# HUBioDataLab/DrugGEN

Hardware: AMD Instinct MI355X
Metric: molecules/sec GAN step (G+D fwd+bwd), N=45 graphs (higher is better)
Workload: dtype f32

## Files before the change

druggen_amd/_lib.py:

```python
from __future__ import annotations

import contextlib
import ctypes
import os
import threading
from ctypes import c_char_p, c_double, c_float, c_int, c_int64, c_size_t, c_void_p

import torch

_PKG = os.path.dirname(os.path.abspath(__file__))
LIB_PATH = os.environ.get("DG_LIB") or os.path.join(_PKG, "lib", "libdruggen_hip.so")

_P = c_void_p


class FFNFwdArgs(ctypes.Structure):
    _fields_ = [(n, _P) for n in ("x", "w1_packed", "b1", "w2_packed", "b2", "gamma", "beta", "y", "h", "relu_bits", "pre_ln",
                                  "mean", "rstd")] + [("R", c_int64), ("eps", c_float)]


class FFNBwdArgs(ctypes.Structure):
    _fields_ = [(n, _P) for n in ("x", "h", "relu_bits", "pre_ln", "mean", "rstd", "gamma", "w1_dgrad_packed", "w2_dgrad_packed",
                                  "dy", "dz_add", "dz", "dh", "dx", "dgamma", "dbeta", "dw1", "db1", "dw2", "db2", "workspace")] + [
        ("workspace_bytes", c_size_t), ("R", c_int64)]


SIGNATURES = {
    "dg_version": (c_int, []),
    "dg_last_error_string": (c_char_p, []),
    "dg_hidden_bytes": (c_size_t, [c_int64, c_int, c_int]),
    "dg_hidden_scale_offset": (c_size_t, [c_int64, c_int]),
    "dg_attn_core_fwd": (c_int, [_P] * 6 + [c_int, c_int, c_int, c_float, c_int, _P]),
    "dg_attn_core_bwd": (c_int, [_P] * 10 + [c_int, c_int, c_int, c_float, c_int, _P]),
    "dg_attn_core_bwd_add": (c_int, [_P] * 11 + [c_int, c_int, c_int, c_float, c_int, _P]),
    "dg_attn_core_bwd2": (c_int, [_P] * 16 + [c_int, c_int, c_int, c_float, c_int, _P]),
    "dg_attn_core_long_workspace_bytes": (c_size_t, [c_int, c_int, c_int]),
    "dg_attn_core_long_fwd": (c_int, [_P] * 6 + [c_int, c_int, c_int, c_float, c_int, _P]),
    "dg_attn_core_long_bwd": (c_int, [_P] * 12 + [c_size_t, c_int, c_int, c_int, c_float, c_int, _P]),
    "dg_attn_core_long_bwd2": (c_int, [_P] * 17 + [c_size_t, c_int, c_int, c_int, c_float, c_int, _P]),
    "dg_attn_half_packed_bytes": (c_size_t, [c_int]),
    "dg_attn_half_pack": (c_int, [_P, _P, _P, c_int, _P]),
    "dg_attn_half_fwd": (c_int, [_P] * 14 + [c_int, c_int, c_int, c_float, c_float, c_int, _P]),
    "dg_attn_half_f32_fwd": (c_int, [_P] * 17 + [c_int, c_int, c_int, c_float, c_float, _P]),
    "dg_attn_half_f32_bwd1_workspace_bytes": (c_size_t, [c_int]),
    "dg_attn_half_f32_bwd1": (c_int, [_P] * 19 + [_P, c_size_t, c_int, c_int, c_int, c_float, _P]),
    "dg_attn_half_bwd_workspace_bytes": (c_size_t, [c_int, c_int]),
    "dg_attn_half_bwd": (c_int, [_P] * 16 + [_P, c_size_t, c_int, c_int, c_int, c_float, c_int, _P]),
    "dg_ln_residual_fwd": (c_int, [_P] * 7 + [c_int64, c_int, c_float, c_int, _P]),
    "dg_ln_workspace_bytes": (c_size_t, [c_int64, c_int]),
    "dg_ln_residual_bwd": (c_int, [_P] * 9 + [_P, c_size_t, c_int64, c_int, c_int, _P]),
    "dg_ln_residual_bwd_add": (c_int, [_P] * 10 + [_P, c_size_t, c_int64, c_int, c_int, _P]),
    "dg_ln_residual_bwd2": (c_int, [_P] * 10 + [_P, c_size_t, c_int64, c_int, c_int, _P]),
    "dg_linear_wgrad_workspace_bytes": (c_size_t, [c_int64, c_int, c_int]),
    "dg_linear_wgrad": (c_int, [_P] * 5 + [_P, c_size_t, c_int64, c_int, c_int, c_int, _P]),
    "dg_row_gemm_packed_bytes": (c_size_t, [c_int, c_int, c_int]),
    "dg_row_gemm_pack": (c_int, [_P, _P, c_int, c_int, c_int, c_int, _P]),
    "dg_row_gemm_mask_words": (c_size_t, [c_int64, c_int, c_int, c_int]),
    "dg_row_gemm": (c_int, [_P] * 3 + [c_int64, c_int, c_int, _P, c_int, _P, _P, _P, _P, _P, _P, _P, _P, c_float, c_int, _P]),
    "dg_linear_wgrad3": (c_int, [_P] * 6 + [_P, c_size_t, c_int64, c_int, _P]),
    "dg_row_gemm_pack3": (c_int, [_P, _P, _P, _P, c_int, c_int, c_int, _P]),
    "dg_row_gemm_lin3": (c_int, [_P] * 5 + [c_int64, _P, _P, _P, c_int, _P]),
    "dg_row_gemm_sum3": (c_int, [_P] * 5 + [c_int64, _P, c_int, _P]),
    "dg_linear_wgrad_batch_begin": (c_int, []),
    "dg_linear_wgrad_batch_end": (c_int, [_P]),
    "dg_launch_pair_begin": (c_int, []),
    "dg_launch_pair_end": (c_int, [_P]),
    "dg_skinny_linear_fwd": (c_int, [_P] * 4 + [c_int64, c_int, c_int, c_int, _P]),
    "dg_skinny_linear_dgrad": (c_int, [_P] * 3 + [c_int64, c_int, c_int, c_int, _P]),
    "dg_skinny_linear_wgrad": (c_int, [_P] * 5 + [c_size_t, c_int64, c_int, c_int, c_int, _P]),
    "dg_embed_node_chain": (c_int, [_P] * 9 + [c_int64, c_int, c_int, _P]),
    "dg_embed_node_bwd": (c_int, [_P] * 8 + [c_int64, c_int, c_int, _P]),
    "dg_head_chain": (c_int, [_P] * 14 + [c_int64, c_int, _P]),
    "dg_head_bwd": (c_int, [_P] * 10 + [c_int64, c_int, _P]),
    "dg_head_wgrad": (c_int, [_P] * 12 + [c_int64, _P]),
    "dg_row_gemm_pack_batch": (c_int, [_P, c_int, c_int, c_int, _P]),
    "dg_row_gemm_ln_bwd_workspace_bytes": (c_size_t, [c_int]),
    "dg_row_gemm_ln_bwd": (c_int, [_P] * 3 + [c_int64, c_int] + [_P] * 7 + [_P, c_size_t, c_int, _P]),
    "dg_row_gemm_ln_bwd_in": (c_int, [_P] * 10 + [_P, c_size_t, c_int64, c_int, c_int, c_int, _P]),
    "dg_edge_ffn_ln_workspace_bytes": (c_size_t, [c_int64, c_int, c_int]),
    "dg_edge_ffn_ln_fwd": (c_int, [_P] * 13 + [c_int64, c_int, c_int, c_float, c_int, _P]),
    "dg_edge_ffn_ln_bwd": (c_int, [_P] * 20 + [_P, c_size_t, c_int64, c_int, c_int, c_int, _P]),
    "dg_edge_ffn_ln_fwd_pair": (c_int, [ctypes.POINTER(FFNFwdArgs), ctypes.POINTER(FFNFwdArgs), c_int, c_int, c_int, _P]),
    "dg_edge_ffn_ln_bwd_pair": (c_int, [ctypes.POINTER(FFNBwdArgs), ctypes.POINTER(FFNBwdArgs), c_int, c_int, c_int, _P]),
    "dg_ffn_f32_packed_bytes": (c_size_t, []),
    "dg_ffn_f32_pack": (c_int, [_P, _P, _P, _P]),
    "dg_ffn_ln_fwd_f32": (c_int, [ctypes.POINTER(FFNFwdArgs), ctypes.POINTER(FFNFwdArgs), _P]),
    "dg_ffn_bf16_padded_rows": (c_int64, [c_int64]),
    "dg_ffn_bf16_packed_bytes": (c_size_t, []),
    "dg_ffn_bf16_pack": (c_int, [_P, _P, _P, _P]),
    "dg_ffn_bf16_mask_words": (c_size_t, [c_int64]),
    "dg_ffn_bf16_workspace_bytes": (c_size_t, [c_int64]),
    "dg_ffn_ln_fwd_bf16": (c_int, [_P] * 11 + [c_int64, c_float, _P]),
    "dg_ffn_ln_bwd_bf16": (c_int, [_P] * 18 + [_P, c_size_t, c_int64, _P]),
    "dg_embed_sym_packed_floats": (c_size_t, []),
    "dg_embed_sym_workspace_bytes": (c_size_t, [c_int, c_int]),
    "dg_embed_sym_dgrad_packed_floats": (c_size_t, []),
    "dg_embed_sym_pack_dgrad": (c_int, [_P, _P, _P]),
    "dg_embed_sym_pack": (c_int, [_P, _P, _P]),
    "dg_embed_sym_fwd": (c_int, [_P] * 6 + [c_int] * 7 + [_P]),
    "dg_embed_sym_bwd": (c_int, [_P] * 12 + [_P, c_size_t] + [c_int] * 7 + [_P]),
    "dg_embed_sym_bwd_bf16_workspace_bytes": (c_size_t, [c_int, c_int]),
    "dg_embed_sym_bwd_bf16": (c_int, [_P] * 11 + [_P, c_size_t] + [c_int] * 6 + [_P]),
    "dg_embed_sym_bwd2": (c_int, [_P] * 11 + [_P, c_size_t] + [c_int] * 7 + [_P]),
    "dg_onehot_embed_workspace_bytes": (c_size_t, [c_int, c_int]),
    "dg_onehot_embed_fwd": (c_int, [_P, _P, _P, c_int, c_int, c_int, c_int, c_int, _P]),
    "dg_onehot_embed_bwd": (c_int, [_P, _P, _P, _P, c_size_t, c_int, c_int, c_int, c_int, c_int, _P]),
    "dg_densify": (c_int, [_P, _P, _P, c_int64, c_int, c_int, c_int, _P, _P, _P, _P]),
    "dg_mol_gather": (c_int, [_P, _P, _P, c_int64, _P, c_int, c_int, c_int, c_int, _P, _P, _P, _P, _P]),
    "dg_adamw_flat": (c_int, [_P, _P, _P, _P, c_int64, c_float, c_float, c_float, c_float, c_float, c_int64, _P]),
    "dg_adamw_flat_devstep": (c_int, [_P, _P, _P, _P, c_int64, c_float, c_float, c_float, c_float, c_float, _P, _P]),
    "dg_argmax_decode": (c_int, [_P, c_int64, c_int, _P, _P]),
    "dg_decode_graph": (c_int, [_P] * 3 + [c_int] * 5 + [_P] * 8 + [_P]),
    "dg_fp_pack": (c_int, [_P, c_int, c_int64, c_int, _P, _P, _P]),
    "dg_fp_tanimoto_workspace_bytes": (c_size_t, [c_int64, c_int64]),
    "dg_fp_tanimoto": (c_int, [_P, _P, c_int64, _P, _P, c_int64, c_int, c_int, _P, _P, _P, c_size_t, _P]),
    "dg_prof_enable": (c_int, [c_int]),
    "dg_prof_reset": (c_int, []),
    "dg_prof_read": (c_int, [c_int, ctypes.POINTER(c_int64), ctypes.POINTER(c_double)]),
    "dg_set_edge_rows": (c_int, [c_int64]),
    "dg_edge_rows": (c_int64, []),
}

KERNEL_IDS = {"attn_fwd": 0, "attn_bwd": 1, "attn_bwd2": 2, "ln_fwd": 3, "ln_bwd": 4, "ln_bwd2": 5, "linear_wgrad": 6, "row_gemm": 7, "embed_sym": 8, "ffn": 9, "ffn_wgrad": 10,
              "attn_half_fwd": 11, "attn_half_bwd": 12,
              "row_gemm_e128": 13, "row_gemm_e_n384": 14, "row_gemm_e_k384": 15,
              "linear_wgrad_e128": 16, "linear_wgrad_e_n384": 17, "linear_wgrad_e_k384": 18,
              "ffn_node": 19, "ffn_wgrad_node": 20, "ffn_f32": 21, "ffn_f32_node": 22}
EDGE_ROWS = 65536
_edge_rows = EDGE_ROWS


def edge_rows() -> int:
    return _edge_rows


def set_edge_rows(rows: int = 0) -> None:
    global _edge_rows
    rows = int(rows) if rows and rows > 0 else EDGE_ROWS
    if rows != _edge_rows:
        check(load().dg_set_edge_rows(rows), "dg_set_edge_rows")
        _edge_rows = rows

_lock = threading.Lock()
_lib = None


class HipExtensionMissing(RuntimeError):
    pass


def load() -> ctypes.CDLL:
    global _lib
    if _lib is not None:
        return _lib
    with _lock:
        if _lib is not None:
            return _lib
        if not os.path.exists(LIB_PATH):
            raise HipExtensionMissing(
                f"{LIB_PATH} not found: build it with `python -m druggen_amd.build` "
                "(druggen_amd has no CPU / eager fallback)")
        lib = ctypes.CDLL(LIB_PATH)
        for name, (res, args) in SIGNATURES.items():
            fn = getattr(lib, name)
            fn.restype, fn.argtypes = res, args
        _lib = lib
        return lib


def check(status: int, what: str) -> None:
    if status != 0:
        msg = load().dg_last_error_string()
        raise RuntimeError(f"{what} failed ({status}): {msg.decode() if msg else '?'}")


def _dev(t):
    if torch.cuda.current_device() == t.device.index:
        return contextlib.nullcontext()
    return torch.cuda.device(t.device)


DTYPES = {torch.float32: 0, torch.bfloat16: 1}
F32_H16 = 2
F32_H24 = 3
F32_DH16, F32_DH24 = 4, 5
F32_H32 = 6
F32_H32_DH16 = 7
HIDDEN_CODES = (F32_H16, F32_H24, F32_H32)


def dt(t) -> int:
    try:
        return DTYPES[t.dtype]
    except KeyError:
        raise RuntimeError(f"druggen_amd kernels store activations as float32 or bfloat16; got {t.dtype}") from None


def ptr(t):
    if t is None:
        return None
    if not t.is_cuda:
        raise RuntimeError("druggen_amd kernels need GPU tensors (no CPU fallback); got device "
                           f"{t.device}")
    if t.dtype not in DTYPES:
        raise RuntimeError(f"druggen_amd kernels are float32 / bfloat16; got {t.dtype}")
    if not t.is_contiguous():
        raise RuntimeError("druggen_amd kernels need contiguous tensors")
    return t.data_ptr()


def fptr(t):
    if t is not None and t.dtype != torch.float32:
        raise RuntimeError(f"expected a float32 tensor, got {t.dtype}")
    return ptr(t)


_raw_stream = getattr(torch._C, "_cuda_getCurrentRawStream", None)


def stream_of(t) -> int:
    if _raw_stream is not None:
        return _raw_stream(t.device.index)
    return torch.cuda.current_stream(t.device).cuda_stream


def launch(name: str, ref, *args) -> None:
    entry = getattr(load(), name)
    with _dev(ref):
        status = entry(*args, stream_of(ref))
    if status != 0:
        check(status, name)


def prof_enable(on=True, kernels=None) -> None:
    if kernels is not None:
        mask = 0
        for k in kernels:
            mask |= 1 << KERNEL_IDS[k]
        if mask & (1 << 31):
            mask -= 1 << 32
    else:
        mask = -1 if on else 0
    check(load().dg_prof_enable(mask), "dg_prof_enable")


def prof_reset() -> None:
    check(load().dg_prof_reset(), "dg_prof_reset")


def prof_read(kernel: str):
    n, ms = c_int64(0), c_double(0.0)
    check(load().dg_prof_read(KERNEL_IDS[kernel], ctypes.byref(n), ctypes.byref(ms)), "dg_prof_read")
    return int(n.value), float(ms.value)
```

druggen_amd/build.py:

```python
from __future__ import annotations

import glob
import os
import shutil
import subprocess
import sys

PKG = os.path.dirname(os.path.abspath(__file__))
CSRC = os.path.join(PKG, "csrc")
LIB_DIR = os.path.join(PKG, "lib")
LIB_PATH = os.path.join(LIB_DIR, "libdruggen_hip.so")
HEADER = os.path.join(os.path.dirname(PKG), "include", "druggen_hip.h")
ARCH = "gfx950"


def sources():
    return sorted(glob.glob(os.path.join(CSRC, "*.hip")))


def _stale() -> bool:
    if not os.path.exists(LIB_PATH):
        return True
    t = os.path.getmtime(LIB_PATH)
    deps = sources() + glob.glob(os.path.join(CSRC, "*.h")) + [HEADER]
    return any(os.path.getmtime(d) > t for d in deps)


def build(force: bool = False, verbose: bool = False) -> str:
    if not force and not _stale():
        return LIB_PATH
    hipcc = shutil.which("hipcc") or "/opt/rocm/bin/hipcc"
    if not os.path.exists(hipcc):
        raise RuntimeError("hipcc not found: cannot build libdruggen_hip.so")
    os.makedirs(LIB_DIR, exist_ok=True)
    objs, jobs = [], []
    headers = glob.glob(os.path.join(CSRC, "*.h")) + [HEADER]
    for src in sources():
        obj = os.path.join(LIB_DIR, os.path.basename(src) + ".o")
        objs.append(obj)
        if (not force and os.path.exists(obj) and os.path.getmtime(obj) > os.path.getmtime(src)
                and all(os.path.getmtime(obj) > os.path.getmtime(h) for h in headers)):
            continue
        jobs.append([hipcc, f"--offload-arch={ARCH}", "-O3", "-std=c++17", "-fPIC", "-ffp-contract=fast",
                     "-c", src, "-o", obj])

    def run(cmd):
        if verbose:
            print(" ".join(cmd), flush=True)
        subprocess.check_call(cmd)

    if jobs:
        from concurrent.futures import ThreadPoolExecutor
        with ThreadPoolExecutor(max_workers=min(len(jobs), os.cpu_count() or 1)) as pool:
            list(pool.map(run, jobs))
    cmd = [hipcc, f"--offload-arch={ARCH}", "-shared", "-fPIC", "-o", LIB_PATH] + objs
    if verbose:
        print(" ".join(cmd), flush=True)
    subprocess.check_call(cmd)
    return LIB_PATH


if __name__ == "__main__":
    print(build(force="--force" in sys.argv, verbose=True))
```

druggen_amd/csrc/embed_sym.hip:

```cpp
#include "bf16.h"
#include "traversal.h"

namespace dg {
void launch_ln_finish(const float* part, int nblocks, int K, int C, float* out0, float* out1, hipStream_t stream);
namespace {

typedef float f32x16 __attribute__((ext_vector_type(16)));

constexpr int kHid = 64;
constexpr int kC = 128;
constexpr int kPairs = 32;
constexpr int kMaxE = 16;
constexpr int kD1Pitch = 68;

enum Act { kRelu = 0, kLeaky = 1, kSigmoid = 2, kTanh = 3 };

template <int act>
__device__ __forceinline__ float act_fwd(float x) {
    switch (act) {
        case kRelu: return fmaxf(x, 0.f);
        case kLeaky: return x > 0.f ? x : 0.01f * x;
        case kSigmoid: return 1.0f / (1.0f + __expf(-x));
        default: return tanhf(x);
    }
}
template <int act>
__device__ __forceinline__ float act_grad_from_output(float y) {
    switch (act) {
        case kRelu: return y > 0.f ? 1.f : 0.f;
        case kLeaky: return y > 0.f ? 1.f : 0.01f;
        case kSigmoid: return y * (1.f - y);
        default: return 1.f - y * y;
    }
}

struct PairTile {
    int b;
    int p0;
};

__device__ __forceinline__ void pair_to_ij(int p, int N, int* i_out, int* j_out) {
    int i = 0;
    while (p >= N - i) {
        p -= N - i;
        ++i;
    }
    *i_out = i;
    *j_out = i + p;
}

template <bool BACKWARD>
struct Smem {
    int ij[kPairs][2];
    float a[64][kMaxE];
    float h1[64 * kHid];
};

template <int EP, int ACT>
__device__ __forceinline__ void stage_tile(const float* __restrict__ a, const float* __restrict__ w1,
                                           const float* __restrict__ b1, int N, int E, int NP, PairTile t,
                                           int (*ij)[2], float (*at)[kMaxE], float* h1) {
    int tid = threadIdx.x;
    asm volatile("" : "+v"(tid));
    if (tid < kPairs) {
        const int p = t.p0 + tid;
        int i = 0, j = 0;
        if (p < NP) pair_to_ij(p, N, &i, &j);
        ij[tid][0] = p < NP ? i : -1;
        ij[tid][1] = j;
    }
    __syncthreads();
    for (int idx = tid; idx < 64 * EP; idx += 256) {
        const int row = idx / EP, e = idx % EP;
        const int pr = row & 31;
        const int i = ij[pr][0], j = ij[pr][1];
        float v = 0.f;
        if (i >= 0 && e < E) {
            const int64_t r = (static_cast<int64_t>(t.b) * N + (row < 32 ? i : j)) * N + (row < 32 ? j : i);
            v = a[r * E + e];
        }
        at[row][e] = v;
    }
    __syncthreads();
    const int u = tid & 63, g = tid >> 6;
    float w[EP];
#pragma unroll
    for (int e = 0; e < EP; ++e) w[e] = e < E ? w1[u * E + e] : 0.f;
    const float bb = b1[u];
    for (int r = 0; r < 16; ++r) {
        const int row = g * 16 + r;
        float s = bb;
#pragma unroll
        for (int e = 0; e < EP; ++e) s = fmaf(w[e], at[row][e], s);
        h1[row * kHid + (((u >> 2) ^ (row & 15)) << 2) + (u & 3)] = act_fwd<ACT>(s);
    }
    __syncthreads();
}

typedef unsigned u32x4e __attribute__((ext_vector_type(4)));
struct Planes { bf16x8 p[3]; };

__device__ __forceinline__ void split2(float x0, float x1, unsigned& h, unsigned& m, unsigned& l) {
    const unsigned a0 = __float_as_uint(x0), a1 = __float_as_uint(x1);
    h = __builtin_amdgcn_perm(a1, a0, 0x07060302u);
    const float r0 = x0 - __uint_as_float(a0 & 0xFFFF0000u), r1 = x1 - __uint_as_float(a1 & 0xFFFF0000u);
    const unsigned b0 = __float_as_uint(r0), b1 = __float_as_uint(r1);
    m = __builtin_amdgcn_perm(b1, b0, 0x07060302u);
    const float s0 = r0 - __uint_as_float(b0 & 0xFFFF0000u), s1 = r1 - __uint_as_float(b1 & 0xFFFF0000u);
    l = __builtin_amdgcn_perm(__float_as_uint(s1), __float_as_uint(s0), 0x07060302u);
}
__device__ __forceinline__ Planes split8(const float (&v)[8]) {
    u32x4e h, m, l;
#pragma unroll
    for (int i = 0; i < 4; ++i) {
        unsigned hh, mm, ll;
        split2(v[2 * i], v[2 * i + 1], hh, mm, ll);
        h[i] = hh;
        m[i] = mm;
        l[i] = ll;
    }
    Planes r;
    r.p[0] = __builtin_bit_cast(bf16x8, h);
    r.p[1] = __builtin_bit_cast(bf16x8, m);
    r.p[2] = __builtin_bit_cast(bf16x8, l);
    return r;
}
__device__ __forceinline__ Planes split8(const float4& a, const float4& b) {
    const float v[8] = {a.x, a.y, a.z, a.w, b.x, b.y, b.z, b.w};
    return split8(v);
}
__device__ __forceinline__ f32x16 mfma6(const Planes& a, const Planes& b, f32x16 c) {
    constexpr int TA[6] = {2, 1, 0, 1, 0, 0}, TB[6] = {0, 1, 2, 0, 1, 0};
#pragma unroll
    for (int t = 0; t < 6; ++t) c = __builtin_amdgcn_mfma_f32_32x32x16_bf16(a.p[TA[t]], b.p[TB[t]], c, 0, 0, 0);
    return c;
}
__device__ __forceinline__ f32x16 mfma_bwd(const Planes& a, const Planes& b, f32x16 c) {
    constexpr int TA[3] = {1, 0, 0}, TB[3] = {0, 1, 0};
#pragma unroll
    for (int t = 0; t < 3; ++t) c = __builtin_amdgcn_mfma_f32_32x32x16_bf16(a.p[TA[t]], b.p[TB[t]], c, 0, 0, 0);
    return c;
}
__device__ __forceinline__ Planes frag_row(const float* tile, int row, int c, int pitch) {
    const float4 a = ld4(tile + row * pitch + ((c ^ (row & 15)) << 2));
    const float4 b = ld4(tile + row * pitch + (((c + 1) ^ (row & 15)) << 2));
    return split8(a, b);
}
__device__ __forceinline__ Planes load_planes(const bf16x8* p) {
    Planes r;
#pragma unroll
    for (int q = 0; q < 3; ++q) r.p[q] = p[q * 64];
    return r;
}

__device__ __forceinline__ void layer2_mfma(const float* h1, const bf16x8* w2f, int lane, f32x16& acc0, f32x16& acc1) {
    const int half = lane >> 5, col = lane & 31;
#pragma unroll
    for (int i = 0; i < 16; ++i) acc0[i] = acc1[i] = 0.f;
#pragma unroll
    for (int ks = 0; ks < 4; ++ks) {
        const Planes b = load_planes(w2f + ks * 3 * 64);
        const Planes a0 = frag_row(h1, col, 4 * ks + 2 * half, kHid);
        const Planes a1 = frag_row(h1, 32 + col, 4 * ks + 2 * half, kHid);
        acc0 = mfma6(a0, b, acc0);
        acc1 = mfma6(a1, b, acc1);
    }
}

__global__ void embed_pack3_kernel(const float* __restrict__ w2, bf16x8* __restrict__ p, int dgrad) {
    const int KS = dgrad ? 8 : 4, NT = dgrad ? 2 : 4;
    const int idx = blockIdx.x * blockDim.x + threadIdx.x;
    if (idx >= NT * KS * 64) return;
    const int lane = idx & 63, ks = (idx >> 6) % KS, t = (idx >> 6) / KS;
    const int n = 32 * t + (lane & 31);
    float v[8];
#pragma unroll
    for (int j = 0; j < 8; ++j) {
        const int k = 16 * ks + 8 * (lane >> 5) + j;
        v[j] = dgrad ? w2[static_cast<size_t>(k) * kHid + n] : w2[static_cast<size_t>(n) * kHid + k];
    }
    const Planes pl = split8(v);
#pragma unroll
    for (int q = 0; q < 3; ++q) p[(static_cast<size_t>(t * KS + ks) * 3 + q) * 64 + lane] = pl.p[q];
}

template <typename T>
__device__ __forceinline__ void store_pair_rows(const float* xt, const int (*ij)[2], int b, int N, T* __restrict__ out,
                                                int tid) {
    const int hw = tid >> 5, l32 = tid & 31;
#pragma unroll
    for (int it = 0; it < 4; ++it) {
        const int pr = hw + 8 * it;
        const int i = ij[pr][0], j = ij[pr][1];
        if (i < 0) continue;
        const float4 v = ld4(xt + pr * kC + 4 * l32);
        const int64_t base = static_cast<int64_t>(b) * N;
        st4(out + ((base + i) * N + j) * kC + 4 * l32, v);
        if (i != j) st4(out + ((base + j) * N + i) * kC + 4 * l32, v);
    }
}

template <typename T, int EP, int ACT>
__global__ __launch_bounds__(256) void embed_sym_fwd_kernel(const float* __restrict__ a, const float* __restrict__ w1,
                                                          const float* __restrict__ b1,
                                                          const float* __restrict__ w2p,
                                                          const float* __restrict__ b2, T* __restrict__ out,
                                                          int B, int N, int E, int tiles_per_mol) {
    __shared__ int ij[kPairs][2];
    __shared__ float at[64][kMaxE];
    __shared__ __attribute__((aligned(16))) float h1[64 * kHid];
    __shared__ __attribute__((aligned(16))) float xt[kPairs * kC];
    const int lane = threadIdx.x & 63, w = __builtin_amdgcn_readfirstlane(threadIdx.x >> 6);
    const int half = lane >> 5, col = lane & 31;
    const int NP = N * (N + 1) / 2;
    const bf16x8* w2f = reinterpret_cast<const bf16x8*>(w2p) + static_cast<size_t>(w) * 4 * 3 * 64 + lane;
    const int n = 32 * w + col;
    const float bias2 = b2[n];
    const int total = B * tiles_per_mol;
    for (int tix = blockIdx.x; tix < total; tix += gridDim.x) {
        const PairTile t{tix / tiles_per_mol, (tix % tiles_per_mol) * kPairs};
        stage_tile<EP, ACT>(a, w1, b1, N, E, NP, t, ij, at, h1);
        f32x16 acc0, acc1;
        layer2_mfma(h1, w2f, lane, acc0, acc1);
#pragma unroll
        for (int reg = 0; reg < 16; ++reg) {
            const int pr = (reg & 3) + 8 * (reg >> 2) + 4 * half;
            xt[pr * kC + n] = 0.5f * (act_fwd<ACT>(acc0[reg] + bias2) + act_fwd<ACT>(acc1[reg] + bias2));
        }
        __syncthreads();
        store_pair_rows(xt, ij, t.b, N, out, static_cast<int>(threadIdx.x));
        __syncthreads();
    }
}

__device__ __forceinline__ void aw2_stage(const float* d2, const float* hq, int n, int col, int half, f32x16 (&aw2)[2]) {
    const int c = n >> 2;
#pragma unroll
    for (int ks = 0; ks < 4; ++ks) {
        float av[8], b0[8], b1v[8];
#pragma unroll
        for (int j = 0; j < 8; ++j) {
            const int r = 16 * ks + 8 * half + j;
            av[j] = d2[r * kC + (((c & ~15) | ((c & 15) ^ (r & 15))) << 2) + (n & 3)];
            b0[j] = hq[r * kHid + ((((col) >> 2) ^ (r & 15)) << 2) + (col & 3)];
            b1v[j] = hq[r * kHid + ((((32 + col) >> 2) ^ (r & 15)) << 2) + (col & 3)];
        }
        const Planes pa = split8(av);
        aw2[0] = mfma_bwd(pa, split8(b0), aw2[0]);
        aw2[1] = mfma_bwd(pa, split8(b1v), aw2[1]);
    }
}
__device__ __forceinline__ f32x16 dh_stage(const float* d2, const bf16x8* w2g, int row, int half) {
    f32x16 d0, d1v;
#pragma unroll
    for (int i = 0; i < 16; ++i) d0[i] = d1v[i] = 0.f;
#pragma unroll
    for (int ks = 0; ks < 8; ks += 2) {
        d0 = mfma_bwd(frag_row(d2, row, 4 * ks + 2 * half, kC), load_planes(w2g + ks * 3 * 64), d0);
        d1v = mfma_bwd(frag_row(d2, row, 4 * (ks + 1) + 2 * half, kC), load_planes(w2g + (ks + 1) * 3 * 64), d1v);
    }
#pragma unroll
    for (int i = 0; i < 16; ++i) d0[i] += d1v[i];
    return d0;
}

struct BwdPart {
    static constexpr int kW2 = 0, kB2 = kC * kHid, kW1 = kB2 + kC, kB1 = kW1 + kHid * kMaxE, kTotal = kB1 + kHid;
};

template <typename T, int EP, int ACT, bool DA>
__global__ __launch_bounds__(256, 2) void embed_sym_bwd_kernel(
    const float* __restrict__ a, const float* __restrict__ w1, const float* __restrict__ b1,
    const float* __restrict__ w2p, const float* __restrict__ w2d, const float* __restrict__ b2,
    const T* __restrict__ g, float* __restrict__ da, float* __restrict__ part, int B, int N, int E,
    int tiles_per_mol) {
    extern __shared__ __attribute__((aligned(16))) char smem_raw[];
    float* h1 = reinterpret_cast<float*>(smem_raw);
    float* d2 = h1 + 64 * kHid;
    float* d1 = d2 + 64 * kC;
    float(*at)[kMaxE] = reinterpret_cast<float(*)[kMaxE]>(d1 + 64 * kD1Pitch);
    int(*ij)[2] = reinterpret_cast<int(*)[2]>(&at[64][0]);
    float4* w1p = reinterpret_cast<float4*>(&ij[kPairs][0]);
    float* gst = d1;
    const int tid = threadIdx.x, lane = tid & 63, w = __builtin_amdgcn_readfirstlane(tid >> 6);
    if (DA) {
        const int u = tid >> 2, eg = tid & 3;
        float v[4];
#pragma unroll
        for (int q = 0; q < 4; ++q) v[q] = eg + 4 * q < E ? w1[u * E + eg + 4 * q] : 0.f;
        w1p[tid] = make_float4(v[0], v[1], v[2], v[3]);
    }

    const int half = lane >> 5, col = lane & 31;
    const int NP = N * (N + 1) / 2;
    const int ut = w & 1, mt = w >> 1;
    const int n = 32 * w + col;
    const float bias2 = b2[n];
    f32x16 aw2[2];
#pragma unroll
    for (int i = 0; i < 16; ++i) aw2[0][i] = aw2[1][i] = 0.f;
    float ab2 = 0.f, ab1 = 0.f, aw1[EP];
#pragma unroll
    for (int e = 0; e < EP; ++e) aw1[e] = 0.f;
    const int total = B * tiles_per_mol;
#ifdef DG_EMBED_DBG
    unsigned long long tl = __builtin_amdgcn_s_memtime(), ts[8] = {0, 0, 0, 0, 0, 0, 0, 0}, t00 = tl;
#define ESTAMP(i) { const unsigned long long t_ = __builtin_amdgcn_s_memtime(); ts[i] += t_ - tl; tl = t_; }
#else
#define ESTAMP(i)
#endif
    for (int tix = blockIdx.x; tix < total; tix += gridDim.x) {
        const PairTile t{tix / tiles_per_mol, (tix % tiles_per_mol) * kPairs};
        stage_tile<EP, ACT>(a, w1, b1, N, E, NP, t, ij, at, h1);
        ESTAMP(0)
        int lo = lane;
        asm volatile("" : "+v"(lo));
        const int half = lo >> 5, col = lo & 31, n = 32 * w + col;
        typedef typename raw4<T>::type Raw;
        Raw gr[4][2];
        {
            const int hw = lo >> 5 | (w << 1), l32 = lo & 31;
#pragma unroll
            for (int it = 0; it < 4; ++it) {
                const int pr = hw + 8 * it;
                const int i = ij[pr][0], j = ij[pr][1];
                const int64_t base = static_cast<int64_t>(t.b) * N;
                const int ii = i >= 0 ? i : 0, jj = i >= 0 ? j : 0;
                gr[it][0] = ld_raw(g + ((base + ii) * N + jj) * kC + 4 * l32);
                gr[it][1] = ld_raw(g + ((base + jj) * N + ii) * kC + 4 * l32);
            }
        }
        f32x16 acc0, acc1;
        layer2_mfma(h1, reinterpret_cast<const bf16x8*>(w2p) + static_cast<size_t>(w) * 4 * 3 * 64 + lo, lo, acc0, acc1);
        {
            const int hw = lo >> 5 | (w << 1), l32 = lo & 31;
#pragma unroll
            for (int it = 0; it < 4; ++it) {
                const int pr = hw + 8 * it;
                const bool diag = ij[pr][0] == ij[pr][1];
                const float4 v = (diag ? 0.25f : 0.5f) * (cvt_raw(gr[it][0]) + cvt_raw(gr[it][1]));
                st4(gst + pr * kC + 4 * l32, ij[pr][0] >= 0 ? v : f4(0.f));
            }
        }
        __syncthreads();
        ESTAMP(1)
#pragma unroll
        for (int reg = 0; reg < 16; ++reg) {
            const int pr = (reg & 3) + 8 * (reg >> 2) + 4 * half;
            const int i = ij[pr][0], j = ij[pr][1];
            float p0 = 0.f, p1 = 0.f;
            if (i >= 0) {
                const float gs = gst[pr * kC + n];
                p0 = gs * act_grad_from_output<ACT>(act_fwd<ACT>(acc0[reg] + bias2));
                p1 = gs * act_grad_from_output<ACT>(act_fwd<ACT>(acc1[reg] + bias2));
            }
            (void)j;
            ab2 += p0 + p1;
            const int c = n >> 2;
            d2[pr * kC + (((c & ~15) | ((c & 15) ^ (pr & 15))) << 2) + (n & 3)] = p0;
            d2[(32 + pr) * kC + (((c & ~15) | ((c & 15) ^ (pr & 15))) << 2) + (n & 3)] = p1;
        }
        __syncthreads();
        ESTAMP(2)
        aw2_stage(d2, h1, n, col, half, aw2);
        ESTAMP(3)
        const f32x16 dh = dh_stage(d2, reinterpret_cast<const bf16x8*>(w2d) + static_cast<size_t>(ut) * 8 * 3 * 64 + lo, 32 * mt + col, half);
        ESTAMP(4)
        const int u = 32 * ut + col;
#pragma unroll
        for (int reg = 0; reg < 16; ++reg) {
            const int row = 32 * mt + (reg & 3) + 8 * (reg >> 2) + 4 * half;
            const float hv = h1[row * kHid + (((u >> 2) ^ (row & 15)) << 2) + (u & 3)];
            const float p = dh[reg] * act_grad_from_output<ACT>(hv);
            ab1 += p;
            float av[EP];
#pragma unroll
            for (int e4 = 0; e4 < EP; e4 += 4) {
                const float4 t4 = ld4(&at[row][e4]);
                av[e4] = t4.x; av[e4 + 1] = t4.y; av[e4 + 2] = t4.z; av[e4 + 3] = t4.w;
            }
#pragma unroll
            for (int e = 0; e < EP; ++e) aw1[e] = fmaf(p, av[e], aw1[e]);
            if (DA) d1[row * kD1Pitch + u] = p;
        }
        ESTAMP(5)
        if (DA) {
            __syncthreads();
            const int row = lo, eg = w;
            float s[4] = {0.f, 0.f, 0.f, 0.f};
#pragma unroll 4
            for (int u4 = 0; u4 < kHid; u4 += 4) {
                const float4 dv = ld4(d1 + row * kD1Pitch + u4);
                const float dvv[4] = {dv.x, dv.y, dv.z, dv.w};
#pragma unroll
                for (int uu = 0; uu < 4; ++uu) {
                    const float4 wv = w1p[(u4 + uu) * 4 + eg];
                    s[0] = fmaf(dvv[uu], wv.x, s[0]);
                    s[1] = fmaf(dvv[uu], wv.y, s[1]);
                    s[2] = fmaf(dvv[uu], wv.z, s[2]);
                    s[3] = fmaf(dvv[uu], wv.w, s[3]);
                }
            }
            const int pr = row & 31;
            const int i = ij[pr][0], j = ij[pr][1];
#pragma unroll
            for (int q = 0; q < 4; ++q) {
                const float other = __shfl_xor(s[q], 32, 64);
                const int e = eg + 4 * q;
                if (i < 0 || e >= E || (row >= 32 && i == j)) continue;
                const int64_t r = (static_cast<int64_t>(t.b) * N + (row < 32 ? i : j)) * N + (row < 32 ? j : i);
                da[r * E + e] = i == j ? s[q] + other : s[q];
            }
        }
        __syncthreads();
        ESTAMP(6)
    }
#ifdef DG_EMBED_DBG
    if (lane == 0 && blockIdx.x == 17) {
        unsigned long long* o = reinterpret_cast<unsigned long long*>(part + static_cast<size_t>(gridDim.x + 1) * BwdPart::kTotal) + 8 * w;
        for (int i = 0; i < 7; ++i) o[i] = ts[i];
        o[7] = __builtin_amdgcn_s_memtime() - t00;
    }
#endif
    float* pw = part + static_cast<size_t>(blockIdx.x) * BwdPart::kTotal;
#pragma unroll
    for (int t2 = 0; t2 < 2; ++t2)
#pragma unroll
        for (int reg = 0; reg < 16; ++reg) {
            const int nn = 32 * w + (reg & 3) + 8 * (reg >> 2) + 4 * half;
            pw[BwdPart::kW2 + nn * kHid + 32 * t2 + col] = aw2[t2][reg];
        }
    ab2 += __shfl_xor(ab2, 32, 64);
    if (half == 0) pw[BwdPart::kB2 + n] = ab2;
    __syncthreads();
    float* red = d2;
    {
        float* slot = red + ((w * 2 + half) * 32 + col) * (kMaxE + 1);
#pragma unroll
        for (int e = 0; e < kMaxE; ++e) slot[e] = e < EP ? aw1[e < EP ? e : 0] : 0.f;
        slot[kMaxE] = ab1;
    }
    __syncthreads();
    for (int idx = tid; idx < kHid * (kMaxE + 1); idx += 256) {
        const int uu = idx / (kMaxE + 1), e = idx % (kMaxE + 1);
        const int utile = uu >> 5, c = uu & 31;
        float s = 0.f;
        for (int mm = 0; mm < 2; ++mm)
            for (int hh = 0; hh < 2; ++hh) s += red[(((utile + 2 * mm) * 2 + hh) * 32 + c) * (kMaxE + 1) + e];
        if (e < kMaxE)
            pw[BwdPart::kW1 + uu * kMaxE + e] = s;
        else
            pw[BwdPart::kB1 + uu] = s;
    }
}

template <typename T, int EP, int ACT>
__global__ __launch_bounds__(256, 2) void embed_sym_bwd2_kernel(
    const float* __restrict__ a, const float* __restrict__ w1, const float* __restrict__ b1,
    const float* __restrict__ w2p, const float* __restrict__ w2d, const float* __restrict__ b2,
    const T* __restrict__ g, const float* __restrict__ tadj, T* __restrict__ gg, float* __restrict__ part, int B, int N,
    int E, int tiles_per_mol) {
    extern __shared__ __attribute__((aligned(16))) char smem_raw[];
    float* h1 = reinterpret_cast<float*>(smem_raw);
    float* d2 = h1 + 64 * kHid;
    float* hb = d2 + 64 * kC;
    float(*at)[kMaxE] = reinterpret_cast<float(*)[kMaxE]>(hb + 64 * kHid);
    float(*tt)[kMaxE] = reinterpret_cast<float(*)[kMaxE]>(&at[64][0]);
    int(*ij)[2] = reinterpret_cast<int(*)[2]>(&tt[64][0]);
    float* gst = reinterpret_cast<float*>(&ij[kPairs][0]);
    const int lane = threadIdx.x & 63, w = __builtin_amdgcn_readfirstlane(threadIdx.x >> 6);
    const int NP = N * (N + 1) / 2;
    const int ut = w & 1, mt = w >> 1;
    f32x16 aw2[2];
#pragma unroll
    for (int i = 0; i < 16; ++i) aw2[0][i] = aw2[1][i] = 0.f;
    float aw1[EP];
#pragma unroll
    for (int e = 0; e < EP; ++e) aw1[e] = 0.f;
    const int total = B * tiles_per_mol;
    for (int tix = blockIdx.x; tix < total; tix += gridDim.x) {
        const PairTile t{tix / tiles_per_mol, (tix % tiles_per_mol) * kPairs};
        stage_tile<EP, ACT>(a, w1, b1, N, E, NP, t, ij, at, h1);
        int tid = threadIdx.x;
        asm volatile("" : "+v"(tid));
        for (int idx = tid; idx < 64 * EP; idx += 256) {
            const int row = idx / EP, e = idx % EP;
            const int pr = row & 31;
            const int i = ij[pr][0], j = ij[pr][1];
            float v = 0.f;
            if (i >= 0 && e < E) {
                const int64_t r = (static_cast<int64_t>(t.b) * N + (row < 32 ? i : j)) * N + (row < 32 ? j : i);
                v = tadj[r * E + e];
            }
            tt[row][e] = v;
        }
        __syncthreads();
        {
            const int u = tid & 63, gq = tid >> 6;
            float wv[EP];
#pragma unroll
            for (int e = 0; e < EP; ++e) wv[e] = e < E ? w1[u * E + e] : 0.f;
            for (int r = 0; r < 16; ++r) {
                const int row = gq * 16 + r;
                float sacc = 0.f;
#pragma unroll
                for (int e = 0; e < EP; ++e) sacc = fmaf(wv[e], tt[row][e], sacc);
                const int o = row * kHid + (((u >> 2) ^ (row & 15)) << 2) + (u & 3);
                hb[o] = sacc * act_grad_from_output<ACT>(h1[o]);
            }
        }
        __syncthreads();
        int lo = lane;
        asm volatile("" : "+v"(lo));
        const int half = lo >> 5, col = lo & 31, n = 32 * w + col;
        const float bias2 = b2[n];
        typedef typename raw4<T>::type Raw;
        Raw gr[4][2];
        {
            const int hw = lo >> 5 | (w << 1), l32 = lo & 31;
#pragma unroll
            for (int it = 0; it < 4; ++it) {
                const int pr = hw + 8 * it;
                const int i = ij[pr][0], j = ij[pr][1];
                const int64_t base = static_cast<int64_t>(t.b) * N;
                const int ii = i >= 0 ? i : 0, jj = i >= 0 ? j : 0;
                gr[it][0] = ld_raw(g + ((base + ii) * N + jj) * kC + 4 * l32);
                gr[it][1] = ld_raw(g + ((base + jj) * N + ii) * kC + 4 * l32);
            }
        }
        f32x16 acc0, acc1, q0, q1;
        {
            const bf16x8* w2f = reinterpret_cast<const bf16x8*>(w2p) + static_cast<size_t>(w) * 4 * 3 * 64 + lo;
            layer2_mfma(h1, w2f, lo, acc0, acc1);
            layer2_mfma(hb, w2f, lo, q0, q1);
        }
        {
            const int hw = lo >> 5 | (w << 1), l32 = lo & 31;
#pragma unroll
            for (int it = 0; it < 4; ++it) {
                const int pr = hw + 8 * it;
                const bool diag = ij[pr][0] == ij[pr][1];
                const float4 v = (diag ? 0.25f : 0.5f) * (cvt_raw(gr[it][0]) + cvt_raw(gr[it][1]));
                st4(gst + pr * kC + 4 * l32, ij[pr][0] >= 0 ? v : f4(0.f));
            }
        }
        __syncthreads();
#pragma unroll
        for (int reg = 0; reg < 16; ++reg) {
            const int pr = (reg & 3) + 8 * (reg >> 2) + 4 * half;
            const int i = ij[pr][0], j = ij[pr][1];
            float p0 = 0.f, p1 = 0.f;
            if (i >= 0) {
                const float gs = gst[pr * kC + n];
                const float d0 = act_grad_from_output<ACT>(act_fwd<ACT>(acc0[reg] + bias2));
                const float d1v = act_grad_from_output<ACT>(act_fwd<ACT>(acc1[reg] + bias2));
                p0 = gs * d0;
                p1 = gs * d1v;
                gst[pr * kC + n] = 0.5f * (q0[reg] * d0 + q1[reg] * d1v);
            }
            (void)j;
            const int c = n >> 2;
            d2[pr * kC + (((c & ~15) | ((c & 15) ^ (pr & 15))) << 2) + (n & 3)] = p0;
            d2[(32 + pr) * kC + (((c & ~15) | ((c & 15) ^ (pr & 15))) << 2) + (n & 3)] = p1;
        }
        __syncthreads();
        store_pair_rows(gst, ij, t.b, N, gg, tid);
        aw2_stage(d2, hb, n, col, half, aw2);
        const f32x16 dh = dh_stage(d2, reinterpret_cast<const bf16x8*>(w2d) + static_cast<size_t>(ut) * 8 * 3 * 64 + lo, 32 * mt + col, half);
        const int u = 32 * ut + col;
#pragma unroll
        for (int reg = 0; reg < 16; ++reg) {
            const int row = 32 * mt + (reg & 3) + 8 * (reg >> 2) + 4 * half;
            const float hv = h1[row * kHid + (((u >> 2) ^ (row & 15)) << 2) + (u & 3)];
            const float p = dh[reg] * act_grad_from_output<ACT>(hv);
            float av[EP];
#pragma unroll
            for (int e4 = 0; e4 < EP; e4 += 4) {
                const float4 t4 = ld4(&tt[row][e4]);
                av[e4] = t4.x; av[e4 + 1] = t4.y; av[e4 + 2] = t4.z; av[e4 + 3] = t4.w;
            }
#pragma unroll
            for (int e = 0; e < EP; ++e) aw1[e] = fmaf(p, av[e], aw1[e]);
        }
        __syncthreads();
    }
    const int half = lane >> 5, col = lane & 31;
    float* pw = part + static_cast<size_t>(blockIdx.x) * BwdPart::kTotal;
#pragma unroll
    for (int t2 = 0; t2 < 2; ++t2)
#pragma unroll
        for (int reg = 0; reg < 16; ++reg) {
            const int nn = 32 * w + (reg & 3) + 8 * (reg >> 2) + 4 * half;
            pw[BwdPart::kW2 + nn * kHid + 32 * t2 + col] = aw2[t2][reg];
        }
    __syncthreads();
    float* red = d2;
    {
        float* slot = red + ((w * 2 + half) * 32 + col) * kMaxE;
#pragma unroll
        for (int e = 0; e < kMaxE; ++e) slot[e] = e < EP ? aw1[e < EP ? e : 0] : 0.f;
    }
    __syncthreads();
    for (int idx = threadIdx.x; idx < kHid * kMaxE; idx += 256) {
        const int uu = idx / kMaxE, e = idx % kMaxE;
        const int utile = uu >> 5, c = uu & 31;
        float sum = 0.f;
        for (int mm = 0; mm < 2; ++mm)
            for (int hh = 0; hh < 2; ++hh) sum += red[(((utile + 2 * mm) * 2 + hh) * 32 + c) * kMaxE + e];
        pw[BwdPart::kW1 + uu * kMaxE + e] = sum;
    }
}

__global__ __launch_bounds__(1024) void embed_finish_kernel(const float* __restrict__ part, int S, float* __restrict__ dw1,
                                                          float* __restrict__ db1, float* __restrict__ dw2,
                                                          float* __restrict__ db2, int E) {
    __shared__ float red[32][33];
    const int c = blockIdx.x * 32 + (threadIdx.x & 31);
    const int g = threadIdx.x >> 5;
    float s = 0.f;
    if (c < BwdPart::kTotal) {
        const float* src = part + c;
        int b = g;
        for (; b + 7 * 32 < S; b += 8 * 32) {
            float v[8];
#pragma unroll
            for (int u = 0; u < 8; ++u) v[u] = src[static_cast<size_t>(b + 32 * u) * BwdPart::kTotal];
            s += ((v[0] + v[1]) + (v[2] + v[3])) + ((v[4] + v[5]) + (v[6] + v[7]));
        }
        for (; b < S; b += 32) s += src[static_cast<size_t>(b) * BwdPart::kTotal];
    }
    red[g][threadIdx.x & 31] = s;
    __syncthreads();
    if (g == 0 && c < BwdPart::kTotal) {
        float t = 0.f;
        for (int i = 0; i < 32; ++i) t += red[i][threadIdx.x];
        if (c >= BwdPart::kW2 && c < BwdPart::kW2 + kC * kHid) dw2[c - BwdPart::kW2] = t;
        else if (c >= BwdPart::kB2 && c < BwdPart::kB2 + kC) { if (db2) db2[c - BwdPart::kB2] = t; }
        else if (c >= BwdPart::kW1 && c < BwdPart::kW1 + kHid * kMaxE) {
            const int i = c - BwdPart::kW1;
            if (i % kMaxE < E) dw1[(i / kMaxE) * E + i % kMaxE] = t;
        } else if (c >= BwdPart::kB1 && c < BwdPart::kB1 + kHid) { if (db1) db1[c - BwdPart::kB1] = t; }
    }
}

template <typename T>
__global__ __launch_bounds__(256) void onehot_embed_fwd_kernel(const int* __restrict__ labels, const float* __restrict__ table,
                                                             T* __restrict__ out, int64_t rows, int N, int E) {
    __shared__ float4 tab[kMaxE * kC / 4];
    for (int i = threadIdx.x; i < E * kC / 4; i += 256) tab[i] = ld4(table + i * 4);
    __syncthreads();
    const int col = threadIdx.x & 31;
    const int64_t NN = static_cast<int64_t>(N) * N;
    for (int64_t r = static_cast<int64_t>(blockIdx.x) * 8 + (threadIdx.x >> 5); r < rows; r += static_cast<int64_t>(gridDim.x) * 8) {
        const int64_t b = r / NN;
        const int ij = static_cast<int>(r - b * NN), i = ij / N, j = ij - i * N;
        int l1 = labels[r], l2 = labels[b * NN + static_cast<int64_t>(j) * N + i];
        l1 = l1 < 0 ? 0 : (l1 >= E ? E - 1 : l1);
        l2 = l2 < 0 ? 0 : (l2 >= E ? E - 1 : l2);
        st4_stream(out + r * kC + 4 * col, 0.5f * (tab[l1 * (kC / 4) + col] + tab[l2 * (kC / 4) + col]));
    }
}

template <typename T, int EP>
__global__ __launch_bounds__(256) void onehot_embed_bwd_kernel(const int* __restrict__ labels, const T* __restrict__ g,
                                                             float* __restrict__ part, int64_t rows, int N, int E) {
    __shared__ float4 red[8][EP][32];
    const int col = threadIdx.x & 31, rp = threadIdx.x >> 5;
    const int64_t NN = static_cast<int64_t>(N) * N;
    float4 acc[EP];
#pragma unroll
    for (int c = 0; c < EP; ++c) acc[c] = f4(0.f);
    for (int64_t r = static_cast<int64_t>(blockIdx.x) * 8 + rp; r < rows; r += static_cast<int64_t>(gridDim.x) * 8) {
        const int64_t b = r / NN;
        const int ij = static_cast<int>(r - b * NN), i = ij / N, j = ij - i * N;
        const int l1 = labels[r], l2 = labels[b * NN + static_cast<int64_t>(j) * N + i];
        const float4 gv = ld4_stream(g + r * kC + 4 * col);
#pragma unroll
        for (int c = 0; c < EP; ++c) {
            const float wgt = 0.5f * ((l1 == c ? 1.f : 0.f) + (l2 == c ? 1.f : 0.f));
            acc[c] = fma4(f4(wgt), gv, acc[c]);
        }
    }
#pragma unroll
    for (int c = 0; c < EP; ++c) red[rp][c][col] = acc[c];
    __syncthreads();
    for (int idx = threadIdx.x; idx < E * 32; idx += 256) {
        const int c = idx >> 5, cc = idx & 31;
        float4 t = f4(0.f);
        for (int p = 0; p < 8; ++p) t += red[p][c][cc];
        st4(part + (static_cast<size_t>(blockIdx.x) * E + c) * kC + 4 * cc, t);
    }
}

constexpr int kOneHotBlocks = 1024;

constexpr int kBwdPerCu = 2;
int embed_grid(int total_tiles, int per_cu) {
    const int cap = 256 * per_cu;
    return total_tiles < cap ? (total_tiles < 1 ? 1 : total_tiles) : cap;
}

bool embed_shape_ok(int N, int E, int H, int C, int act) {
    return N >= 1 && E >= 1 && E <= kMaxE && H == kHid && C == kC && act >= 0 && act <= 3;
}

}
}

using namespace dg;

extern "C" size_t dg_embed_sym_packed_floats(void) { return static_cast<size_t>(4) * 4 * 3 * 64 * 4; }

extern "C" size_t dg_embed_sym_workspace_bytes(int B, int N) {
    const int tiles = B * ((N * (N + 1) / 2 + kPairs - 1) / kPairs);
    return (static_cast<size_t>(embed_grid(tiles, kBwdPerCu)) + 1) * BwdPart::kTotal * sizeof(float) + 256;
}

extern "C" int dg_embed_sym_pack(const float* w2, float* packed, dg_stream_t stream_) {
    if (!w2 || !packed) return fail(DG_E_ARG, "dg_embed_sym_pack: null pointer");
    hipLaunchKernelGGL(embed_pack3_kernel, dim3(4), dim3(256), 0, static_cast<hipStream_t>(stream_), w2,
                       reinterpret_cast<bf16x8*>(packed), 0);
    return check_launch("dg_embed_sym_pack");
}

extern "C" size_t dg_embed_sym_dgrad_packed_floats(void) { return static_cast<size_t>(2) * 8 * 3 * 64 * 4; }

extern "C" int dg_embed_sym_pack_dgrad(const float* w2, float* packed, dg_stream_t stream_) {
    if (!w2 || !packed) return fail(DG_E_ARG, "dg_embed_sym_pack_dgrad: null pointer");
    hipLaunchKernelGGL(embed_pack3_kernel, dim3(4), dim3(256), 0, static_cast<hipStream_t>(stream_), w2,
                       reinterpret_cast<bf16x8*>(packed), 1);
    return check_launch("dg_embed_sym_pack_dgrad");
}

extern "C" int dg_embed_sym_fwd(const float* a, const float* w1, const float* b1, const float* w2_packed,
                                const float* b2, void* out, int B, int N, int E, int H, int C, int act, int dtype,
                                dg_stream_t stream_) {
    if (!a || !w1 || !b1 || !w2_packed || !b2 || !out) return fail(DG_E_ARG, "dg_embed_sym_fwd: null pointer");
    if (!dtype_ok(dtype)) return fail(DG_E_ARG, "dg_embed_sym_fwd: unknown dtype %d", dtype);
    if (B < 0 || !embed_shape_ok(N, E, H, C, act))
        return fail(DG_E_SHAPE, "dg_embed_sym_fwd: unsupported N=%d E=%d H=%d C=%d act=%d (need E<=16, H=64, C=128)", N, E,
                    H, C, act);
    if (B == 0) return 0;
    hipStream_t stream = static_cast<hipStream_t>(stream_);
    const int tpm = (N * (N + 1) / 2 + kPairs - 1) / kPairs;
    ProfScope prof(DG_K_EMBED_SYM, stream);
    note_forward(static_cast<int64_t>(B) * N * N);
#define FWD_A(T, EP_, ACT_)                                                                                      \
    hipLaunchKernelGGL((embed_sym_fwd_kernel<T, EP_, ACT_>), dim3(embed_grid(B * tpm, 8)), dim3(256), 0, stream, a, w1, \
                       b1, w2_packed, b2, static_cast<T*>(out), B, N, E, tpm);
#define FWD(T, EP_)                                                                                             \
    switch (act) {                                                                                              \
        case kRelu: FWD_A(T, EP_, kRelu) break;                                                                 \
        case kLeaky: FWD_A(T, EP_, kLeaky) break;                                                               \
        case kSigmoid: FWD_A(T, EP_, kSigmoid) break;                                                           \
        default: FWD_A(T, EP_, kTanh) break;                                                                    \
    }
    if (dtype == DG_DTYPE_BF16) {
        if (E <= 8) { FWD(bf16_t, 8) } else { FWD(bf16_t, 16) }
    } else {
        if (E <= 8) { FWD(float, 8) } else { FWD(float, 16) }
    }
#undef FWD_A
#undef FWD
    return check_launch("dg_embed_sym_fwd");
}

extern "C" int dg_embed_sym_bwd(const float* a, const float* w1, const float* b1, const float* w2_packed,
                                const float* w2_dgrad_packed, const float* b2, const void* g, float* da, float* dw1,
                                float* db1, float* dw2, float* db2, void* workspace, size_t workspace_bytes, int B,
                                int N, int E, int H, int C, int act, int dtype, dg_stream_t stream_) {
    if (!a || !w1 || !b1 || !w2_packed || !w2_dgrad_packed || !b2 || !g || !dw1 || !db1 || !dw2 || !db2 || !workspace)
        return fail(DG_E_ARG, "dg_embed_sym_bwd: null pointer");
    if (!dtype_ok(dtype)) return fail(DG_E_ARG, "dg_embed_sym_bwd: unknown dtype %d", dtype);
    if (B < 1 || !embed_shape_ok(N, E, H, C, act))
        return fail(DG_E_SHAPE, "dg_embed_sym_bwd: unsupported B=%d N=%d E=%d H=%d C=%d act=%d", B, N, E, H, C, act);
    if (workspace_bytes < dg_embed_sym_workspace_bytes(B, N))
        return fail(DG_E_WORKSPACE, "dg_embed_sym_bwd: workspace too small");
    hipStream_t stream = static_cast<hipStream_t>(stream_);
    const int tpm = (N * (N + 1) / 2 + kPairs - 1) / kPairs;
    const int grid = embed_grid(B * tpm, kBwdPerCu);
    float* part = static_cast<float*>(workspace);
    constexpr int lds_bytes = (64 * kHid + 64 * kC + 64 * kD1Pitch + 64 * kMaxE + kHid * 16) * 4 + kPairs * 2 * 4;
    ProfScope prof(DG_K_EMBED_SYM, stream);
    note_forward(static_cast<int64_t>(B) * N * N);
#define BWD_D(T, EP_, ACT_, DA_)                                                                                  \
    {                                                                                                             \
        DG_OPT_IN_LDS((&embed_sym_bwd_kernel<T, EP_, ACT_, DA_>), lds_bytes);                                      \
        hipLaunchKernelGGL((embed_sym_bwd_kernel<T, EP_, ACT_, DA_>), dim3(grid), dim3(256), lds_bytes, stream, a, \
                           w1, b1, w2_packed, w2_dgrad_packed, b2, static_cast<const T*>(g), da, part, B, N, E, tpm); \
    }
#define BWD_A(T, EP_, ACT_)                                                                                       \
    {                                                                                                             \
        if (da) BWD_D(T, EP_, ACT_, true) else BWD_D(T, EP_, ACT_, false)                                         \
    }
#define BWD(T, EP_)                                                                                               \
    switch (act) {                                                                                                \
        case kRelu: BWD_A(T, EP_, kRelu) break;                                                                   \
        case kLeaky: BWD_A(T, EP_, kLeaky) break;                                                                 \
        case kSigmoid: BWD_A(T, EP_, kSigmoid) break;                                                             \
        default: BWD_A(T, EP_, kTanh) break;                                                                      \
    }
    if (dtype == DG_DTYPE_BF16) {
        if (E <= 8) BWD(bf16_t, 8) else BWD(bf16_t, 16)
    } else {
        if (E <= 8) BWD(float, 8) else BWD(float, 16)
    }
#undef BWD_A
#undef BWD_D
#undef BWD
    hipLaunchKernelGGL(embed_finish_kernel, dim3((BwdPart::kTotal + 31) / 32), dim3(1024), 0, stream, part, grid, dw1, db1, dw2,
                       db2, E);
    return check_launch("dg_embed_sym_bwd");
}

extern "C" int dg_embed_sym_bwd2(const float* a, const float* w1, const float* b1, const float* w2_packed,
                                 const float* w2_dgrad_packed, const float* b2, const void* g, const float* t, void* gg,
                                 float* gw1, float* gw2, void* workspace, size_t workspace_bytes, int B, int N, int E,
                                 int H, int C, int act, int dtype, dg_stream_t stream_) {
    if (!a || !w1 || !b1 || !w2_packed || !w2_dgrad_packed || !b2 || !g || !t || !gg || !gw1 || !gw2 || !workspace)
        return fail(DG_E_ARG, "dg_embed_sym_bwd2: null pointer");
    if (!dtype_ok(dtype)) return fail(DG_E_ARG, "dg_embed_sym_bwd2: unknown dtype %d", dtype);
    if (act != kRelu && act != kLeaky)
        return fail(DG_E_ARG, "dg_embed_sym_bwd2: only piecewise-linear activations (relu, leaky) have this closed form");
    if (B < 1 || !embed_shape_ok(N, E, H, C, act))
        return fail(DG_E_SHAPE, "dg_embed_sym_bwd2: unsupported B=%d N=%d E=%d H=%d C=%d act=%d", B, N, E, H, C, act);
    if (workspace_bytes < dg_embed_sym_workspace_bytes(B, N))
        return fail(DG_E_WORKSPACE, "dg_embed_sym_bwd2: workspace too small");
    hipStream_t stream = static_cast<hipStream_t>(stream_);
    const int tpm = (N * (N + 1) / 2 + kPairs - 1) / kPairs;
    const int grid = embed_grid(B * tpm, kBwdPerCu);
    float* part = static_cast<float*>(workspace);
    constexpr int lds_bytes = (64 * kHid + 64 * kC + 64 * kHid + 2 * 64 * kMaxE + kPairs * kC) * 4 + kPairs * 2 * 4;
    ProfScope prof(DG_K_EMBED_SYM, stream);
    note_forward(static_cast<int64_t>(B) * N * N);
#define BWD2_A(T, EP_, ACT_)                                                                                       \
    {                                                                                                              \
        DG_OPT_IN_LDS((&embed_sym_bwd2_kernel<T, EP_, ACT_>), lds_bytes);                                           \
        hipLaunchKernelGGL((embed_sym_bwd2_kernel<T, EP_, ACT_>), dim3(grid), dim3(256), lds_bytes, stream, a, w1,  \
                           b1, w2_packed, w2_dgrad_packed, b2, static_cast<const T*>(g), t, static_cast<T*>(gg),   \
                           part, B, N, E, tpm);                                                                    \
    }
#define BWD2(T, EP_)                                                     \
    if (act == kRelu) BWD2_A(T, EP_, kRelu) else BWD2_A(T, EP_, kLeaky)
    if (dtype == DG_DTYPE_BF16) {
        if (E <= 8) BWD2(bf16_t, 8) else BWD2(bf16_t, 16)
    } else {
        if (E <= 8) BWD2(float, 8) else BWD2(float, 16)
    }
#undef BWD2
#undef BWD2_A
    hipLaunchKernelGGL(embed_finish_kernel, dim3((BwdPart::kTotal + 31) / 32), dim3(1024), 0, stream, part, grid, gw1,
                       static_cast<float*>(nullptr), gw2, static_cast<float*>(nullptr), E);
    return check_launch("dg_embed_sym_bwd2");
}

extern "C" size_t dg_onehot_embed_workspace_bytes(int E, int C) {
    return E >= 1 && E <= kMaxE && C == kC ? static_cast<size_t>(kOneHotBlocks) * E * C * sizeof(float) : 0;
}

extern "C" int dg_onehot_embed_fwd(const int* labels, const float* table, void* out, int B, int N, int E, int C, int dtype,
                                   dg_stream_t stream_) {
    if (!labels || !table || !out) return fail(DG_E_ARG, "dg_onehot_embed_fwd: null pointer");
    if (!dtype_ok(dtype)) return fail(DG_E_ARG, "dg_onehot_embed_fwd: unknown dtype %d", dtype);
    if (B < 0 || N < 1 || E < 1 || E > kMaxE || C != kC)
        return fail(DG_E_SHAPE, "dg_onehot_embed_fwd: unsupported N=%d E=%d C=%d (need E<=16, C=128)", N, E, C);
    if (B == 0) return 0;
    hipStream_t stream = static_cast<hipStream_t>(stream_);
    const int64_t rows = static_cast<int64_t>(B) * N * N;
    const int grid = static_cast<int>(rows / 8 + 1 < 4096 ? rows / 8 + 1 : 4096);
    ProfScope prof(DG_K_EMBED_SYM, stream);
    note_forward(static_cast<int64_t>(B) * N * N);
    if (dtype == DG_DTYPE_BF16)
        hipLaunchKernelGGL((onehot_embed_fwd_kernel<bf16_t>), dim3(grid), dim3(256), 0, stream, labels, table,
                           static_cast<bf16_t*>(out), rows, N, E);
    else
        hipLaunchKernelGGL((onehot_embed_fwd_kernel<float>), dim3(grid), dim3(256), 0, stream, labels, table,
                           static_cast<float*>(out), rows, N, E);
    return check_launch("dg_onehot_embed_fwd");
}

extern "C" int dg_onehot_embed_bwd(const int* labels, const void* g, float* dtable, void* workspace, size_t workspace_bytes,
                                   int B, int N, int E, int C, int dtype, dg_stream_t stream_) {
    if (!labels || !g || !dtable || !workspace) return fail(DG_E_ARG, "dg_onehot_embed_bwd: null pointer");
    if (!dtype_ok(dtype)) return fail(DG_E_ARG, "dg_onehot_embed_bwd: unknown dtype %d", dtype);
    if (B < 1 || N < 1 || E < 1 || E > kMaxE || C != kC)
        return fail(DG_E_SHAPE, "dg_onehot_embed_bwd: unsupported B=%d N=%d E=%d C=%d", B, N, E, C);
    if (workspace_bytes < dg_onehot_embed_workspace_bytes(E, C)) return fail(DG_E_WORKSPACE, "dg_onehot_embed_bwd: workspace too small");
    hipStream_t stream = static_cast<hipStream_t>(stream_);
    const int64_t rows = static_cast<int64_t>(B) * N * N;
    const int grid = static_cast<int>(rows / 8 + 1 < kOneHotBlocks ? rows / 8 + 1 : kOneHotBlocks);
    float* part = static_cast<float*>(workspace);
    ProfScope prof(DG_K_EMBED_SYM, stream);
    note_forward(static_cast<int64_t>(B) * N * N);
#define BWD(T, EP_)                                                                                         \
    hipLaunchKernelGGL((onehot_embed_bwd_kernel<T, EP_>), dim3(grid), dim3(256), 0, stream, labels,          \
                       static_cast<const T*>(g), part, rows, N, E);
    if (dtype == DG_DTYPE_BF16) {
        if (E <= 8) { BWD(bf16_t, 8) } else { BWD(bf16_t, 16) }
    } else {
        if (E <= 8) { BWD(float, 8) } else { BWD(float, 16) }
    }
#undef BWD
    launch_ln_finish(part, grid, 1, E * C, dtable, nullptr, stream);
    return check_launch("dg_onehot_embed_bwd");
}
```

druggen_amd/functional/embed.py:

```python
from __future__ import annotations

import torch
from torch.autograd import Function
from torch.autograd.function import once_differentiable

from .. import _lib
from ..options import options
from ._runtime import _account, _c, in_second_order_forward, _inputs_only, PackCache, _scratch
from .dense import _double_backward_fallback, linear


_ACT_IDS = {"relu": 0, "leaky": 1, "sigmoid": 2, "tanh": 3}
_ACT_FNS = {"relu": torch.relu, "leaky": lambda t: torch.nn.functional.leaky_relu(t, 0.01),
            "sigmoid": torch.sigmoid, "tanh": torch.tanh}


_embed_pack_cache = PackCache(1024)


def _embed_packed_w2(w2, dgrad: bool = False):
    def make(w2):
        lib = _lib.load()
        n_floats = lib.dg_embed_sym_dgrad_packed_floats() if dgrad else lib.dg_embed_sym_packed_floats()
        packed = torch.empty(int(n_floats), dtype=torch.float32, device=w2.device)
        wd = _c(w2.detach())
        _lib.launch("dg_embed_sym_pack_dgrad" if dgrad else "dg_embed_sym_pack", w2, _lib.ptr(wd), _lib.ptr(packed))
        return packed
    return _embed_pack_cache.get((w2,), (dgrad,), make)


def _composite_embed_sym(a, w1, b1, w2, b2, act):
    f = _ACT_FNS[act]
    h = f(linear(a, w1, b1))
    e = f(linear(h, w2, b2))
    return (e + e.permute(0, 2, 1, 3)) / 2


class OutSlot:
    __slots__ = ("tensor",)

    def __init__(self, tensor):
        self.tensor = tensor


def _take_slot(slot, shape, dtype, device):
    if slot is None:
        return torch.empty(*shape, dtype=dtype, device=device)
    t = slot.tensor
    if tuple(t.shape) != tuple(shape) or t.dtype != dtype or t.device != device or not t.is_contiguous():
        raise RuntimeError("OutSlot does not match the embedding's output")
    return t.view(shape)


class _JoinParts(Function):

    @staticmethod
    def forward(ctx, slot, *parts):
        ctx.sizes = [p.shape[0] for p in parts]
        off = 0
        for p_ in parts:
            if p_.data_ptr() != slot.tensor[off:off + p_.shape[0]].data_ptr():
                raise RuntimeError("join_parts: a part does not live in its slice of the buffer")
            off += p_.shape[0]
        return slot.tensor.view(slot.tensor.shape)

    @staticmethod
    def backward(ctx, g):
        outs, off = [], 0
        for n in ctx.sizes:
            outs.append(g[off:off + n])
            off += n
        return (None, *outs)


def join_parts(slot, parts):
    return _JoinParts.apply(slot, *parts)


class _EmbedSym(Function):
    @staticmethod
    def forward(ctx, a, w1, b1, w2, b2, act, out_dtype, slot=None):
        a = _c(a)
        B, N, _, E = a.shape
        H, C = w1.shape[0], w2.shape[0]
        out = _take_slot(slot, (B, N, N, C), out_dtype, a.device)
        _lib.launch("dg_embed_sym_fwd", a, _lib.fptr(a), _lib.fptr(_c(w1)), _lib.fptr(_c(b1)),
                    _lib.fptr(_embed_packed_w2(w2)), _lib.fptr(_c(b2)), _lib.ptr(out), B, N, E, H, C, _ACT_IDS[act],
                    _lib.dt(out))
        _account("embed_sym", B * N * N * (4 * E + out.element_size() * C), 2 * B * N * N * (E * H + H * C))
        ctx.save_for_backward(a, w1, b1, w2, b2)
        ctx.act = act
        ctx.out_dtype = out_dtype
        return out

    @staticmethod
    def backward(ctx, g):
        a, w1, b1, w2, b2 = ctx.saved_tensors
        act = ctx.act
        if torch.is_grad_enabled():
            odt = ctx.out_dtype
            if act in _PIECEWISE_LINEAR:
                outs = _EmbedSymBwd.apply(a, w1, b1, w2, b2, g, act, odt, ctx.needs_input_grad[0],
                                          ctx.needs_input_grad[1] and not _inputs_only())
                return tuple(outs) + (None, None, None)
            return _double_backward_fallback(lambda *t: _composite_embed_sym(*t, act).to(odt), (a, w1, b1, w2, b2), g) + (None, None, None)
        return _embed_bwd_launch(a, w1, b1, w2, b2, g, act, ctx.out_dtype, ctx.needs_input_grad[0],
                                 ctx.needs_input_grad[1] and not _inputs_only()) + (None, None, None)


_PIECEWISE_LINEAR = ("relu", "leaky")


def _embed_bwd_launch(a, w1, b1, w2, b2, g, act, out_dtype, need_da, need_w):
    B, N, _, E = a.shape
    H, C = w1.shape[0], w2.shape[0]
    lib = _lib.load()
    g = _c(g if g.dtype == out_dtype else g.to(out_dtype))
    da = torch.empty_like(a) if need_da else None
    dw1, db1, dw2, db2 = (torch.empty_like(t) for t in (w1, b1, w2, b2))
    if (out_dtype == torch.bfloat16 and act in _PIECEWISE_LINEAR and E <= 8 and N <= 48
            and options.embed_bf16 == "fast"):
        need = int(lib.dg_embed_sym_bwd_bf16_workspace_bytes(B, N))
        ws = _scratch(a, need, "embed16")
        _lib.launch("dg_embed_sym_bwd_bf16", a, _lib.fptr(a), _lib.fptr(_c(w1)), _lib.fptr(_c(b1)), _lib.fptr(_c(w2)),
                    _lib.fptr(_c(b2)), _lib.ptr(g), _lib.ptr(da), _lib.ptr(dw1), _lib.ptr(db1), _lib.ptr(dw2), _lib.ptr(db2),
                    ws.data_ptr(), ws.numel(), B, N, E, H, C, _ACT_IDS[act])
        _account("embed_sym", B * N * N * (4 * E * (2 if da is not None else 1) + 2 * g.element_size() * C),
                 2 * B * N * N * (E * H + H * C) * 3)
        if not need_w:
            dw1 = db1 = dw2 = db2 = None
        return da, dw1, db1, dw2, db2
    need = int(lib.dg_embed_sym_workspace_bytes(B, N))
    ws = _scratch(a, need, "embed")
    _lib.launch("dg_embed_sym_bwd", a, _lib.fptr(a), _lib.fptr(_c(w1)), _lib.fptr(_c(b1)), _lib.fptr(_embed_packed_w2(w2)),
                _lib.fptr(_embed_packed_w2(w2, True)), _lib.fptr(_c(b2)), _lib.ptr(g), _lib.ptr(da), _lib.ptr(dw1),
                _lib.ptr(db1), _lib.ptr(dw2), _lib.ptr(db2), ws.data_ptr(), ws.numel(), B, N, E, H, C, _ACT_IDS[act],
                _lib.dt(g))
    _account("embed_sym", B * N * N * (4 * E * (2 if da is not None else 1) + g.element_size() * C),
             2 * B * N * N * (E * H + H * C) * 3)
    if not need_w:
        dw1 = db1 = dw2 = db2 = None
    return da, dw1, db1, dw2, db2


class _EmbedSymBwd(Function):

    @staticmethod
    def forward(ctx, a, w1, b1, w2, b2, g, act, out_dtype, need_da, need_w):
        ctx.save_for_backward(a, w1, b1, w2, b2, g)
        ctx.act, ctx.out_dtype = act, out_dtype
        outs = _embed_bwd_launch(a.detach(), w1.detach(), b1.detach(), w2.detach(), b2.detach(), g.detach(), act,
                                 out_dtype, need_da, need_w)
        ctx.mark_non_differentiable(*[o for o in outs[1:] if o is not None])
        return outs

    @staticmethod
    @torch.autograd.function.once_differentiable
    def backward(ctx, t_da, t_dw1, t_db1, t_dw2, t_db2):
        a, w1, b1, w2, b2, g = ctx.saved_tensors
        if t_da is None:
            return (None,) * 10
        B, N, _, E = a.shape
        H, C = w1.shape[0], w2.shape[0]
        lib = _lib.load()
        g = _c(g if g.dtype == ctx.out_dtype else g.to(ctx.out_dtype))
        t = _c(t_da.float())
        gg = torch.empty_like(g)
        gw1, gw2 = torch.empty_like(w1), torch.empty_like(w2)
        need = int(lib.dg_embed_sym_workspace_bytes(B, N))
        ws = _scratch(a, need, "embed")
        _lib.launch("dg_embed_sym_bwd2", a, _lib.fptr(_c(a)), _lib.fptr(_c(w1)), _lib.fptr(_c(b1)),
                    _lib.fptr(_embed_packed_w2(w2)), _lib.fptr(_embed_packed_w2(w2, True)), _lib.fptr(_c(b2)), _lib.ptr(g),
                    _lib.fptr(t), _lib.ptr(gg), _lib.ptr(gw1), _lib.ptr(gw2), ws.data_ptr(), ws.numel(), B, N, E, H, C,
                    _ACT_IDS[ctx.act], _lib.dt(g))
        _account("embed_sym", B * N * N * (8 * E + 2 * g.element_size() * C), 2 * B * N * N * (E * H + H * C) * 4)
        if _inputs_only() or not ctx.needs_input_grad[1]:
            gw1 = gw2 = None
        return None, gw1, None, gw2, None, gg, None, None, None, None


def embed_sym(a, w1, b1, w2, b2, act: str, out_dtype=torch.float32, slot=None):
    ok = (a.is_cuda and a.dtype == torch.float32 and a.dim() == 4 and a.shape[1] == a.shape[2] and act in _ACT_IDS
          and a.shape[-1] <= 16 and tuple(w1.shape) == (64, a.shape[-1]) and tuple(w2.shape) == (128, 64)
          and b1 is not None and b2 is not None)
    if not ok or (in_second_order_forward() and act not in _PIECEWISE_LINEAR):
        out = _composite_embed_sym(a, w1, b1, w2, b2, act).to(out_dtype)
        if slot is not None:
            slot.tensor = None
        return out
    return _EmbedSym.apply(a, w1, b1, w2, b2, act, out_dtype, slot)


def as_one_hot(a, labels=None):
    if not (torch.is_tensor(a) and a.is_cuda and a.dim() == 4):
        return a
    if getattr(a, "_dg_labels", None) is not None and getattr(a, "_dg_labels_version", None) == a._version:
        return a
    a._dg_labels_version = a._version
    if a.requires_grad or a.dtype != torch.float32:
        a._dg_labels = False
        return a
    with torch.no_grad():
        if labels is None:
            labels = a.argmax(-1).to(torch.int32)
        ok = ((a.amax(-1) == 1) & (a.sum(-1) == 1) & (a.amin(-1) == 0)).all() if a.shape[-1] > 1 else (a == 1).all()
    a._dg_labels = labels.contiguous() if bool(ok) else False
    return a


def attach_one_hot_labels(a, labels):
    if labels.dtype != torch.int32 or tuple(labels.shape) != tuple(a.shape[:-1]) or labels.device != a.device:
        raise ValueError("labels must be an int32 tensor on a's device with a's shape minus the last dim")
    a._dg_labels = labels if labels.is_contiguous() else labels.contiguous()
    a._dg_labels_version = a._version
    return a


def one_hot_labels(a):
    lab = getattr(a, "_dg_labels", None)
    if not torch.is_tensor(lab) or getattr(a, "_dg_labels_version", None) != a._version:
        return None
    return lab


class _OneHotEmbed(Function):
    @staticmethod
    def forward(ctx, labels, table, out_dtype, slot=None):
        B, N = labels.shape[0], labels.shape[1]
        E, C = table.shape
        table = _c(table)
        out = _take_slot(slot, (B, N, N, C), out_dtype, labels.device)
        _lib.launch("dg_onehot_embed_fwd", labels, labels.data_ptr(), _lib.fptr(table), _lib.ptr(out), B, N, E, C,
                    _lib.dt(out))
        _account("embed_sym", B * N * N * (8 + out.element_size() * C))
        ctx.save_for_backward(labels)
        ctx.shape = (E, C, out_dtype)
        return out

    @staticmethod
    @once_differentiable
    def backward(ctx, g):
        (labels,) = ctx.saved_tensors
        E, C, out_dtype = ctx.shape
        B, N = labels.shape[0], labels.shape[1]
        lib = _lib.load()
        g = _c(g if g.dtype == out_dtype else g.to(out_dtype))
        dtable = torch.empty(E, C, dtype=torch.float32, device=g.device)
        need = int(lib.dg_onehot_embed_workspace_bytes(E, C))
        ws = _scratch(g, need, "onehot")
        _lib.launch("dg_onehot_embed_bwd", g, labels.data_ptr(), _lib.ptr(g), _lib.ptr(dtable), ws.data_ptr(), ws.numel(), B,
                    N, E, C, _lib.dt(g))
        _account("embed_sym", B * N * N * (8 + g.element_size() * C))
        return None, dtable, None, None


def embed_sym_onehot(labels, w1, b1, w2, b2, act: str, out_dtype=torch.float32, slot=None):
    f = _ACT_FNS[act]
    table = f(torch.nn.functional.linear(f(w1.t() + b1), w2, b2))
    return _OneHotEmbed.apply(labels, table, out_dtype, slot)
```

druggen_amd/options.py:

```python
from __future__ import annotations

import contextlib
import os

_CHOICES = {
    "hidden": ("dh16", "dh24", "f32", "f24", "f16"),
    "ffn_f32": ("unfused", "fused"),
    "attn_half_f32": ("fused", "n48", "off"),
    "attn_half_f32_bwd": ("fused", "nograph", "off", "force"),
    "attn_half": ("fused", "unfused", "force"),
    "ffn_bf16": ("fused", "unfused"),
    "low_memory_share": ("auto", "on", "off"),
    "ln_bwd_epilogue": (True, False),
    "ln_bwd_prologue": (True, False),
    "ffn_pair": (True, False),
    "penalty_wgrad": ("joined", "engine"),
    "embed_bf16": ("fast", "general"),
}
_ENV = {"hidden": "DG_HIDDEN", "ffn_f32": "DG_FFN_F32", "attn_half_f32": "DG_ATTN_HALF_F32",
        "attn_half_f32_bwd": "DG_ATTN_HALF_F32_BWD", "attn_half": "DG_ATTN_HALF", "ffn_bf16": "DG_FFN_BF16",
        "low_memory_share": "DG_LOW_MEMORY_SHARE"}


class _Options:
    def __init__(self):
        for name, choices in _CHOICES.items():
            value = choices[0]
            env = _ENV.get(name)
            if env and os.environ.get(env) is not None:
                value = os.environ[env]
                if value not in choices:
                    raise ValueError(f"{env}={value!r}: expected one of {choices}")
            object.__setattr__(self, name, value)

    def __setattr__(self, name, value):
        if name not in _CHOICES:
            raise AttributeError(f"druggen_amd.options has no option {name!r}")
        if value not in _CHOICES[name]:
            raise ValueError(f"options.{name} = {value!r}: expected one of {_CHOICES[name]}")
        object.__setattr__(self, name, value)

    def set(self, **kw):
        for k, v in kw.items():
            setattr(self, k, v)

    @contextlib.contextmanager
    def override(self, **kw):
        prev = {k: getattr(self, k) for k in kw}
        self.set(**kw)
        try:
            yield self
        finally:
            self.set(**prev)

    def as_dict(self):
        return {k: getattr(self, k) for k in _CHOICES}


options = _Options()
```

Measured before the change: 4912.

## Save layer-2 activation sign bits in embed forward and skip recompute in backward

```diff
diff --git a/druggen_amd/_lib.py b/druggen_amd/_lib.py
--- a/druggen_amd/_lib.py
+++ b/druggen_amd/_lib.py
@@ -23,6 +23,18 @@
     _fields_ = [(n, _P) for n in ("x", "h", "relu_bits", "pre_ln", "mean", "rstd", "gamma", "w1_dgrad_packed", "w2_dgrad_packed",
                                   "dy", "dz_add", "dz", "dh", "dx", "dgamma", "dbeta", "dw1", "db1", "dw2", "db2", "workspace")] + [
         ("workspace_bytes", c_size_t), ("R", c_int64)]
+
+
+class EmbedBwdArgs(ctypes.Structure):
+    _fields_ = [(n, _P) for n in ("a", "w1", "b1", "w2_packed", "w2_dgrad_packed", "b2", "g", "sign_bits", "da", "dw1", "db1",
+                                  "dw2", "db2", "workspace")] + [("workspace_bytes", c_size_t)] + [
+        (n, c_int) for n in ("B", "N", "E", "H", "C", "act", "dtype")]
+
+
+class EmbedBwd2Args(ctypes.Structure):
+    _fields_ = [(n, _P) for n in ("a", "w1", "b1", "w2_packed", "w2_dgrad_packed", "b2", "g", "t", "sign_bits", "gg", "gw1",
+                                  "gw2", "workspace")] + [("workspace_bytes", c_size_t)] + [
+        (n, c_int) for n in ("B", "N", "E", "H", "C", "act", "dtype")]
 
 
 SIGNATURES = {
@@ -121,6 +133,13 @@
     "dg_edge_rows": (c_int64, []),
 }
 
+EXT_SIGNATURES = {
+    "dg_embed_sym_sign_words": (c_size_t, [c_int, c_int]),
+    "dg_embed_sym_fwd_bits": (c_int, [_P] * 7 + [c_int] * 7 + [_P]),
+    "dg_embed_sym_bwd_ex": (c_int, [ctypes.POINTER(EmbedBwdArgs), _P]),
+    "dg_embed_sym_bwd2_ex": (c_int, [ctypes.POINTER(EmbedBwd2Args), _P]),
+}
+
 KERNEL_IDS = {"attn_fwd": 0, "attn_bwd": 1, "attn_bwd2": 2, "ln_fwd": 3, "ln_bwd": 4, "ln_bwd2": 5, "linear_wgrad": 6, "row_gemm": 7, "embed_sym": 8, "ffn": 9, "ffn_wgrad": 10,
               "attn_half_fwd": 11, "attn_half_bwd": 12,
               "row_gemm_e128": 13, "row_gemm_e_n384": 14, "row_gemm_e_k384": 15,
@@ -161,7 +180,7 @@
                 f"{LIB_PATH} not found: build it with `python -m druggen_amd.build` "
                 "(druggen_amd has no CPU / eager fallback)")
         lib = ctypes.CDLL(LIB_PATH)
-        for name, (res, args) in SIGNATURES.items():
+        for name, (res, args) in list(SIGNATURES.items()) + list(EXT_SIGNATURES.items()):
             fn = getattr(lib, name)
             fn.restype, fn.argtypes = res, args
         _lib = lib
diff --git a/druggen_amd/build.py b/druggen_amd/build.py
--- a/druggen_amd/build.py
+++ b/druggen_amd/build.py
@@ -11,6 +11,7 @@
 LIB_DIR = os.path.join(PKG, "lib")
 LIB_PATH = os.path.join(LIB_DIR, "libdruggen_hip.so")
 HEADER = os.path.join(os.path.dirname(PKG), "include", "druggen_hip.h")
+HEADER_EXT = os.path.join(os.path.dirname(PKG), "include", "druggen_hip_ext.h")
 ARCH = "gfx950"
 
 
@@ -22,7 +23,7 @@
     if not os.path.exists(LIB_PATH):
         return True
     t = os.path.getmtime(LIB_PATH)
-    deps = sources() + glob.glob(os.path.join(CSRC, "*.h")) + [HEADER]
+    deps = sources() + glob.glob(os.path.join(CSRC, "*.h")) + [HEADER, HEADER_EXT]
     return any(os.path.getmtime(d) > t for d in deps)
 
 
@@ -34,7 +35,7 @@
         raise RuntimeError("hipcc not found: cannot build libdruggen_hip.so")
     os.makedirs(LIB_DIR, exist_ok=True)
     objs, jobs = [], []
-    headers = glob.glob(os.path.join(CSRC, "*.h")) + [HEADER]
+    headers = glob.glob(os.path.join(CSRC, "*.h")) + [HEADER, HEADER_EXT]
     for src in sources():
         obj = os.path.join(LIB_DIR, os.path.basename(src) + ".o")
         objs.append(obj)
diff --git a/druggen_amd/csrc/embed_sym.hip b/druggen_amd/csrc/embed_sym.hip
--- a/druggen_amd/csrc/embed_sym.hip
+++ b/druggen_amd/csrc/embed_sym.hip
@@ -1,5 +1,6 @@
 #include "bf16.h"
 #include "traversal.h"
+#include "../../include/druggen_hip_ext.h"
 
 namespace dg {
 void launch_ln_finish(const float* part, int nblocks, int K, int C, float* out0, float* out1, hipStream_t stream);
@@ -200,11 +201,27 @@
     }
 }
 
-template <typename T, int EP, int ACT>
+constexpr int kSignWordsPerTile = 256;
+__device__ __forceinline__ unsigned sign_word(const f32x16& acc0, const f32x16& acc1, float bias2) {
+    unsigned m = 0;
+#pragma unroll
+    for (int reg = 0; reg < 16; ++reg) {
+        m |= (acc0[reg] + bias2 > 0.f ? 1u : 0u) << reg;
+        m |= (acc1[reg] + bias2 > 0.f ? 1u : 0u) << (16 + reg);
+    }
+    return m;
+}
+template <int act>
+__device__ __forceinline__ float act_grad_from_bit(unsigned word, int bit) {
+    return (word >> bit) & 1u ? 1.f : (act == kRelu ? 0.f : 0.01f);
+}
+
+template <typename T, int EP, int ACT, bool BITS>
 __global__ __launch_bounds__(256) void embed_sym_fwd_kernel(const float* __restrict__ a, const float* __restrict__ w1,
                                                           const float* __restrict__ b1,
                                                           const float* __restrict__ w2p,
                                                           const float* __restrict__ b2, T* __restrict__ out,
+                                                          unsigned* __restrict__ sign_bits,
                                                           int B, int N, int E, int tiles_per_mol) {
     __shared__ int ij[kPairs][2];
     __shared__ float at[64][kMaxE];
@@ -222,6 +239,7 @@
         stage_tile<EP, ACT>(a, w1, b1, N, E, NP, t, ij, at, h1);
         f32x16 acc0, acc1;
         layer2_mfma(h1, w2f, lane, acc0, acc1);
+        if (BITS) sign_bits[static_cast<size_t>(tix) * kSignWordsPerTile + threadIdx.x] = sign_word(acc0, acc1, bias2);
 #pragma unroll
         for (int reg = 0; reg < 16; ++reg) {
             const int pr = (reg & 3) + 8 * (reg >> 2) + 4 * half;
@@ -268,12 +286,12 @@
     static constexpr int kW2 = 0, kB2 = kC * kHid, kW1 = kB2 + kC, kB1 = kW1 + kHid * kMaxE, kTotal = kB1 + kHid;
 };
 
-template <typename T, int EP, int ACT, bool DA>
+template <typename T, int EP, int ACT, bool DA, bool WG, bool BITS>
 __global__ __launch_bounds__(256, 2) void embed_sym_bwd_kernel(
     const float* __restrict__ a, const float* __restrict__ w1, const float* __restrict__ b1,
     const float* __restrict__ w2p, const float* __restrict__ w2d, const float* __restrict__ b2,
-    const T* __restrict__ g, float* __restrict__ da, float* __restrict__ part, int B, int N, int E,
-    int tiles_per_mol) {
+    const T* __restrict__ g, const unsigned* __restrict__ sign_bits, float* __restrict__ da, float* __restrict__ part,
+    int B, int N, int E, int tiles_per_mol) {
     extern __shared__ __attribute__((aligned(16))) char smem_raw[];
     float* h1 = reinterpret_cast<float*>(smem_raw);
     float* d2 = h1 + 64 * kHid;
@@ -331,7 +349,11 @@
             }
         }
         f32x16 acc0, acc1;
-        layer2_mfma(h1, reinterpret_cast<const bf16x8*>(w2p) + static_cast<size_t>(w) * 4 * 3 * 64 + lo, lo, acc0, acc1);
+        unsigned sw = 0;
+        if (BITS)
+            sw = sign_bits[static_cast<size_t>(tix) * kSignWordsPerTile + 64 * w + lo];
+        else
+            layer2_mfma(h1, reinterpret_cast<const bf16x8*>(w2p) + static_cast<size_t>(w) * 4 * 3 * 64 + lo, lo, acc0, acc1);
         {
             const int hw = lo >> 5 | (w << 1), l32 = lo & 31;
 #pragma unroll
@@ -351,18 +373,18 @@
             float p0 = 0.f, p1 = 0.f;
             if (i >= 0) {
                 const float gs = gst[pr * kC + n];
-                p0 = gs * act_grad_from_output<ACT>(act_fwd<ACT>(acc0[reg] + bias2));
-                p1 = gs * act_grad_from_output<ACT>(act_fwd<ACT>(acc1[reg] + bias2));
+                p0 = gs * (BITS ? act_grad_from_bit<ACT>(sw, reg) : act_grad_from_output<ACT>(act_fwd<ACT>(acc0[reg] + bias2)));
+                p1 = gs * (BITS ? act_grad_from_bit<ACT>(sw, 16 + reg) : act_grad_from_output<ACT>(act_fwd<ACT>(acc1[reg] + bias2)));
             }
             (void)j;
-            ab2 += p0 + p1;
+            if (WG) ab2 += p0 + p1;
             const int c = n >> 2;
             d2[pr * kC + (((c & ~15) | ((c & 15) ^ (pr & 15))) << 2) + (n & 3)] = p0;
             d2[(32 + pr) * kC + (((c & ~15) | ((c & 15) ^ (pr & 15))) << 2) + (n & 3)] = p1;
         }
         __syncthreads();
         ESTAMP(2)
-        aw2_stage(d2, h1, n, col, half, aw2);
+        if (WG) aw2_stage(d2, h1, n, col, half, aw2);
         ESTAMP(3)
         const f32x16 dh = dh_stage(d2, reinterpret_cast<const bf16x8*>(w2d) + static_cast<size_t>(ut) * 8 * 3 * 64 + lo, 32 * mt + col, half);
         ESTAMP(4)
@@ -372,15 +394,17 @@
             const int row = 32 * mt + (reg & 3) + 8 * (reg >> 2) + 4 * half;
             const float hv = h1[row * kHid + (((u >> 2) ^ (row & 15)) << 2) + (u & 3)];
             const float p = dh[reg] * act_grad_from_output<ACT>(hv);
-            ab1 += p;
-            float av[EP];
-#pragma unroll
-            for (int e4 = 0; e4 < EP; e4 += 4) {
-                const float4 t4 = ld4(&at[row][e4]);
-                av[e4] = t4.x; av[e4 + 1] = t4.y; av[e4 + 2] = t4.z; av[e4 + 3] = t4.w;
-            }
-#pragma unroll
-            for (int e = 0; e < EP; ++e) aw1[e] = fmaf(p, av[e], aw1[e]);
+            if (WG) {
+                ab1 += p;
+                float av[EP];
+#pragma unroll
+                for (int e4 = 0; e4 < EP; e4 += 4) {
+                    const float4 t4 = ld4(&at[row][e4]);
+                    av[e4] = t4.x; av[e4 + 1] = t4.y; av[e4 + 2] = t4.z; av[e4 + 3] = t4.w;
+                }
+#pragma unroll
+                for (int e = 0; e < EP; ++e) aw1[e] = fmaf(p, av[e], aw1[e]);
+            }
             if (DA) d1[row * kD1Pitch + u] = p;
         }
         ESTAMP(5)
@@ -416,12 +440,13 @@
         ESTAMP(6)
     }
 #ifdef DG_EMBED_DBG
-    if (lane == 0 && blockIdx.x == 17) {
+    if (WG && lane == 0 && blockIdx.x == 17) {
         unsigned long long* o = reinterpret_cast<unsigned long long*>(part + static_cast<size_t>(gridDim.x + 1) * BwdPart::kTotal) + 8 * w;
         for (int i = 0; i < 7; ++i) o[i] = ts[i];
         o[7] = __builtin_amdgcn_s_memtime() - t00;
     }
 #endif
+    if (!WG) return;
     float* pw = part + static_cast<size_t>(blockIdx.x) * BwdPart::kTotal;
 #pragma unroll
     for (int t2 = 0; t2 < 2; ++t2)
@@ -454,12 +479,12 @@
     }
 }
 
-template <typename T, int EP, int ACT>
+template <typename T, int EP, int ACT, bool WG, bool BITS>
 __global__ __launch_bounds__(256, 2) void embed_sym_bwd2_kernel(
     const float* __restrict__ a, const float* __restrict__ w1, const float* __restrict__ b1,
     const float* __restrict__ w2p, const float* __restrict__ w2d, const float* __restrict__ b2,
-    const T* __restrict__ g, const float* __restrict__ tadj, T* __restrict__ gg, float* __restrict__ part, int B, int N,
-    int E, int tiles_per_mol) {
+    const T* __restrict__ g, const float* __restrict__ tadj, const unsigned* __restrict__ sign_bits, T* __restrict__ gg,
+    float* __restrict__ part, int B, int N, int E, int tiles_per_mol) {
     extern __shared__ __attribute__((aligned(16))) char smem_raw[];
     float* h1 = reinterpret_cast<float*>(smem_raw);
     float* d2 = h1 + 64 * kHid;
@@ -529,9 +554,13 @@
             }
         }
         f32x16 acc0, acc1, q0, q1;
+        unsigned sw = 0;
         {
             const bf16x8* w2f = reinterpret_cast<const bf16x8*>(w2p) + static_cast<size_t>(w) * 4 * 3 * 64 + lo;
-            layer2_mfma(h1, w2f, lo, acc0, acc1);
+            if (BITS)
+                sw = sign_bits[static_cast<size_t>(tix) * kSignWordsPerTile + 64 * w + lo];
+            else
+                layer2_mfma(h1, w2f, lo, acc0, acc1);
             layer2_mfma(hb, w2f, lo, q0, q1);
         }
         {
@@ -552,38 +581,45 @@
             float p0 = 0.f, p1 = 0.f;
             if (i >= 0) {
                 const float gs = gst[pr * kC + n];
-                const float d0 = act_grad_from_output<ACT>(act_fwd<ACT>(acc0[reg] + bias2));
-                const float d1v = act_grad_from_output<ACT>(act_fwd<ACT>(acc1[reg] + bias2));
+                const float d0 = BITS ? act_grad_from_bit<ACT>(sw, reg) : act_grad_from_output<ACT>(act_fwd<ACT>(acc0[reg] + bias2));
+                const float d1v = BITS ? act_grad_from_bit<ACT>(sw, 16 + reg) : act_grad_from_output<ACT>(act_fwd<ACT>(acc1[reg] + bias2));
                 p0 = gs * d0;
                 p1 = gs * d1v;
-                gst[pr * kC + n] = 0.5f * (q0[reg] * d0 + q1[reg] * d1v);
+                float x0 = q0[reg] * d0, x1 = q1[reg] * d1v;
+                if (BITS) asm("" : "+v"(x0), "+v"(x1));
+                gst[pr * kC + n] = 0.5f * (x0 + x1);
             }
             (void)j;
-            const int c = n >> 2;
-            d2[pr * kC + (((c & ~15) | ((c & 15) ^ (pr & 15))) << 2) + (n & 3)] = p0;
-            d2[(32 + pr) * kC + (((c & ~15) | ((c & 15) ^ (pr & 15))) << 2) + (n & 3)] = p1;
+            if (WG) {
+                const int c = n >> 2;
+                d2[pr * kC + (((c & ~15) | ((c & 15) ^ (pr & 15))) << 2) + (n & 3)] = p0;
+                d2[(32 + pr) * kC + (((c & ~15) | ((c & 15) ^ (pr & 15))) << 2) + (n & 3)] = p1;
+            }
         }
         __syncthreads();
         store_pair_rows(gst, ij, t.b, N, gg, tid);
-        aw2_stage(d2, hb, n, col, half, aw2);
-        const f32x16 dh = dh_stage(d2, reinterpret_cast<const bf16x8*>(w2d) + static_cast<size_t>(ut) * 8 * 3 * 64 + lo, 32 * mt + col, half);
-        const int u = 32 * ut + col;
-#pragma unroll
-        for (int reg = 0; reg < 16; ++reg) {
-            const int row = 32 * mt + (reg & 3) + 8 * (reg >> 2) + 4 * half;
-            const float hv = h1[row * kHid + (((u >> 2) ^ (row & 15)) << 2) + (u & 3)];
-            const float p = dh[reg] * act_grad_from_output<ACT>(hv);
-            float av[EP];
-#pragma unroll
-            for (int e4 = 0; e4 < EP; e4 += 4) {
-                const float4 t4 = ld4(&tt[row][e4]);
-                av[e4] = t4.x; av[e4 + 1] = t4.y; av[e4 + 2] = t4.z; av[e4 + 3] = t4.w;
-            }
-#pragma unroll
-            for (int e = 0; e < EP; ++e) aw1[e] = fmaf(p, av[e], aw1[e]);
+        if (WG) {
+            aw2_stage(d2, hb, n, col, half, aw2);
+            const f32x16 dh = dh_stage(d2, reinterpret_cast<const bf16x8*>(w2d) + static_cast<size_t>(ut) * 8 * 3 * 64 + lo, 32 * mt + col, half);
+            const int u = 32 * ut + col;
+#pragma unroll
+            for (int reg = 0; reg < 16; ++reg) {
+                const int row = 32 * mt + (reg & 3) + 8 * (reg >> 2) + 4 * half;
+                const float hv = h1[row * kHid + (((u >> 2) ^ (row & 15)) << 2) + (u & 3)];
+                const float p = dh[reg] * act_grad_from_output<ACT>(hv);
+                float av[EP];
+#pragma unroll
+                for (int e4 = 0; e4 < EP; e4 += 4) {
+                    const float4 t4 = ld4(&tt[row][e4]);
+                    av[e4] = t4.x; av[e4 + 1] = t4.y; av[e4 + 2] = t4.z; av[e4 + 3] = t4.w;
+                }
+#pragma unroll
+                for (int e = 0; e < EP; ++e) aw1[e] = fmaf(p, av[e], aw1[e]);
+            }
         }
         __syncthreads();
     }
+    if (!WG) return;
     const int half = lane >> 5, col = lane & 31;
     float* pw = part + static_cast<size_t>(blockIdx.x) * BwdPart::kTotal;
 #pragma unroll
@@ -732,37 +768,169 @@
     return check_launch("dg_embed_sym_pack_dgrad");
 }
 
-extern "C" int dg_embed_sym_fwd(const float* a, const float* w1, const float* b1, const float* w2_packed,
-                                const float* b2, void* out, int B, int N, int E, int H, int C, int act, int dtype,
-                                dg_stream_t stream_) {
-    if (!a || !w1 || !b1 || !w2_packed || !b2 || !out) return fail(DG_E_ARG, "dg_embed_sym_fwd: null pointer");
-    if (!dtype_ok(dtype)) return fail(DG_E_ARG, "dg_embed_sym_fwd: unknown dtype %d", dtype);
+extern "C" size_t dg_embed_sym_sign_words(int B, int N) {
+    if (B < 1 || N < 1) return 0;
+    return static_cast<size_t>(B) * ((N * (N + 1) / 2 + kPairs - 1) / kPairs) * kSignWordsPerTile;
+}
+
+namespace {
+
+bool sign_bits_ok(int act, int dtype) { return (act == kRelu || act == kLeaky) && dtype == DG_DTYPE_F32; }
+
+int embed_fwd_impl(const char* who, const float* a, const float* w1, const float* b1, const float* w2_packed,
+                   const float* b2, void* out, unsigned* sign_bits, int B, int N, int E, int H, int C, int act, int dtype,
+                   dg_stream_t stream_) {
+    if (!a || !w1 || !b1 || !w2_packed || !b2 || !out) return fail(DG_E_ARG, "%s: null pointer", who);
+    if (!dtype_ok(dtype)) return fail(DG_E_ARG, "%s: unknown dtype %d", who, dtype);
     if (B < 0 || !embed_shape_ok(N, E, H, C, act))
-        return fail(DG_E_SHAPE, "dg_embed_sym_fwd: unsupported N=%d E=%d H=%d C=%d act=%d (need E<=16, H=64, C=128)", N, E,
-                    H, C, act);
+        return fail(DG_E_SHAPE, "%s: unsupported N=%d E=%d H=%d C=%d act=%d (need E<=16, H=64, C=128)", who, N, E, H, C, act);
+    if (sign_bits && !sign_bits_ok(act, dtype))
+        return fail(DG_E_ARG, "%s: sign bits exist for relu / leaky and float32 output only", who);
     if (B == 0) return 0;
     hipStream_t stream = static_cast<hipStream_t>(stream_);
     const int tpm = (N * (N + 1) / 2 + kPairs - 1) / kPairs;
     ProfScope prof(DG_K_EMBED_SYM, stream);
     note_forward(static_cast<int64_t>(B) * N * N);
-#define FWD_A(T, EP_, ACT_)                                                                                      \
-    hipLaunchKernelGGL((embed_sym_fwd_kernel<T, EP_, ACT_>), dim3(embed_grid(B * tpm, 8)), dim3(256), 0, stream, a, w1, \
-                       b1, w2_packed, b2, static_cast<T*>(out), B, N, E, tpm);
+#define FWD_A(T, EP_, ACT_, BITS_)                                                                                      \
+    hipLaunchKernelGGL((embed_sym_fwd_kernel<T, EP_, ACT_, BITS_>), dim3(embed_grid(B * tpm, 8)), dim3(256), 0, stream, \
+                       a, w1, b1, w2_packed, b2, static_cast<T*>(out), sign_bits, B, N, E, tpm);
 #define FWD(T, EP_)                                                                                             \
     switch (act) {                                                                                              \
-        case kRelu: FWD_A(T, EP_, kRelu) break;                                                                 \
-        case kLeaky: FWD_A(T, EP_, kLeaky) break;                                                               \
-        case kSigmoid: FWD_A(T, EP_, kSigmoid) break;                                                           \
-        default: FWD_A(T, EP_, kTanh) break;                                                                    \
-    }
-    if (dtype == DG_DTYPE_BF16) {
+        case kRelu: FWD_A(T, EP_, kRelu, false) break;                                                          \
+        case kLeaky: FWD_A(T, EP_, kLeaky, false) break;                                                        \
+        case kSigmoid: FWD_A(T, EP_, kSigmoid, false) break;                                                    \
+        default: FWD_A(T, EP_, kTanh, false) break;                                                             \
+    }
+#define FWD_BITS(EP_)                                                                                           \
+    if (act == kRelu) { FWD_A(float, EP_, kRelu, true) } else { FWD_A(float, EP_, kLeaky, true) }
+    if (sign_bits) {
+        if (E <= 8) { FWD_BITS(8) } else { FWD_BITS(16) }
+    } else if (dtype == DG_DTYPE_BF16) {
         if (E <= 8) { FWD(bf16_t, 8) } else { FWD(bf16_t, 16) }
     } else {
         if (E <= 8) { FWD(float, 8) } else { FWD(float, 16) }
     }
 #undef FWD_A
 #undef FWD
-    return check_launch("dg_embed_sym_fwd");
+#undef FWD_BITS
+    return check_launch(who);
+}
+
+int embed_bwd_impl(const char* who, const dg_embed_bwd_args& x, dg_stream_t stream_) {
+    const int B = x.B, N = x.N, E = x.E, act = x.act, dtype = x.dtype;
+    const bool wg = x.dw1 != nullptr;
+    if (!dtype_ok(dtype)) return fail(DG_E_ARG, "%s: unknown dtype %d", who, dtype);
+    if (B < 1 || !embed_shape_ok(N, E, x.H, x.C, act))
+        return fail(DG_E_SHAPE, "%s: unsupported B=%d N=%d E=%d H=%d C=%d act=%d", who, B, N, E, x.H, x.C, act);
+    if (wg && x.workspace_bytes < dg_embed_sym_workspace_bytes(B, N)) return fail(DG_E_WORKSPACE, "%s: workspace too small", who);
+    if (x.sign_bits && !sign_bits_ok(act, dtype))
+        return fail(DG_E_ARG, "%s: sign bits exist for relu / leaky and float32 gradients only", who);
+    if (!wg && !x.da) return 0;
+    hipStream_t stream = static_cast<hipStream_t>(stream_);
+    const int tpm = (N * (N + 1) / 2 + kPairs - 1) / kPairs;
+    const int grid = embed_grid(B * tpm, kBwdPerCu);
+    float* part = static_cast<float*>(x.workspace);
+    constexpr int lds_bytes = (64 * kHid + 64 * kC + 64 * kD1Pitch + 64 * kMaxE + kHid * 16) * 4 + kPairs * 2 * 4;
+    ProfScope prof(DG_K_EMBED_SYM, stream);
+    note_forward(static_cast<int64_t>(B) * N * N);
+#define BWD_K(T, EP_, ACT_, DA_, WG_, BITS_)                                                                        \
+    {                                                                                                               \
+        DG_OPT_IN_LDS((&embed_sym_bwd_kernel<T, EP_, ACT_, DA_, WG_, BITS_>), lds_bytes);                            \
+        hipLaunchKernelGGL((embed_sym_bwd_kernel<T, EP_, ACT_, DA_, WG_, BITS_>), dim3(grid), dim3(256), lds_bytes,  \
+                           stream, x.a, x.w1, x.b1, x.w2_packed, x.w2_dgrad_packed, x.b2, static_cast<const T*>(x.g), \
+                           x.sign_bits, x.da, part, B, N, E, tpm);                                                  \
+    }
+#define BWD_D(T, EP_, ACT_, BITS_)                                                                                  \
+    {                                                                                                               \
+        if (!wg) BWD_K(T, EP_, ACT_, true, false, BITS_)                                                            \
+        else if (x.da) BWD_K(T, EP_, ACT_, true, true, BITS_)                                                       \
+        else BWD_K(T, EP_, ACT_, false, true, BITS_)                                                                \
+    }
+#define BWD(T, EP_)                                                                                                 \
+    switch (act) {                                                                                                  \
+        case kRelu: BWD_D(T, EP_, kRelu, false) break;                                                              \
+        case kLeaky: BWD_D(T, EP_, kLeaky, false) break;                                                            \
+        case kSigmoid: BWD_D(T, EP_, kSigmoid, false) break;                                                        \
+        default: BWD_D(T, EP_, kTanh, false) break;                                                                 \
+    }
+#define BWD_BITS(EP_)                                                                                               \
+    if (act == kRelu) BWD_D(float, EP_, kRelu, true) else BWD_D(float, EP_, kLeaky, true)
+    if (x.sign_bits) {
+        if (E <= 8) BWD_BITS(8) else BWD_BITS(16)
+    } else if (dtype == DG_DTYPE_BF16) {
+        if (E <= 8) BWD(bf16_t, 8) else BWD(bf16_t, 16)
+    } else {
+        if (E <= 8) BWD(float, 8) else BWD(float, 16)
+    }
+#undef BWD_K
+#undef BWD_D
+#undef BWD
+#undef BWD_BITS
+    if (wg)
+        hipLaunchKernelGGL(embed_finish_kernel, dim3((BwdPart::kTotal + 31) / 32), dim3(1024), 0, stream, part, grid, x.dw1,
+                           x.db1, x.dw2, x.db2, E);
+    return check_launch(who);
+}
+
+int embed_bwd2_impl(const char* who, const dg_embed_bwd2_args& x, dg_stream_t stream_) {
+    const int B = x.B, N = x.N, E = x.E, act = x.act, dtype = x.dtype;
+    const bool wg = x.gw1 != nullptr;
+    if (!dtype_ok(dtype)) return fail(DG_E_ARG, "%s: unknown dtype %d", who, dtype);
+    if (act != kRelu && act != kLeaky)
+        return fail(DG_E_ARG, "%s: only piecewise-linear activations (relu, leaky) have this closed form", who);
+    if (B < 1 || !embed_shape_ok(N, E, x.H, x.C, act))
+        return fail(DG_E_SHAPE, "%s: unsupported B=%d N=%d E=%d H=%d C=%d act=%d", who, B, N, E, x.H, x.C, act);
+    if (wg && x.workspace_bytes < dg_embed_sym_workspace_bytes(B, N)) return fail(DG_E_WORKSPACE, "%s: workspace too small", who);
+    if (x.sign_bits && !sign_bits_ok(act, dtype))
+        return fail(DG_E_ARG, "%s: sign bits exist for relu / leaky and float32 gradients only", who);
+    hipStream_t stream = static_cast<hipStream_t>(stream_);
+    const int tpm = (N * (N + 1) / 2 + kPairs - 1) / kPairs;
+    const int grid = embed_grid(B * tpm, kBwdPerCu);
+    float* part = static_cast<float*>(x.workspace);
+    constexpr int lds_bytes = (64 * kHid + 64 * kC + 64 * kHid + 2 * 64 * kMaxE + kPairs * kC) * 4 + kPairs * 2 * 4;
+    ProfScope prof(DG_K_EMBED_SYM, stream);
+    note_forward(static_cast<int64_t>(B) * N * N);
+#define BWD2_K(T, EP_, ACT_, WG_, BITS_)                                                                             \
+    {                                                                                                                \
+        DG_OPT_IN_LDS((&embed_sym_bwd2_kernel<T, EP_, ACT_, WG_, BITS_>), lds_bytes);                                 \
+        hipLaunchKernelGGL((embed_sym_bwd2_kernel<T, EP_, ACT_, WG_, BITS_>), dim3(grid), dim3(256), lds_bytes, stream, \
+                           x.a, x.w1, x.b1, x.w2_packed, x.w2_dgrad_packed, x.b2, static_cast<const T*>(x.g), x.t,     \
+                           x.sign_bits, static_cast<T*>(x.gg), part, B, N, E, tpm);                                  \
+    }
+#define BWD2_A(T, EP_, ACT_, BITS_)                                                                                  \
+    {                                                                                                                \
+        if (wg) BWD2_K(T, EP_, ACT_, true, BITS_) else BWD2_K(T, EP_, ACT_, false, BITS_)                            \
+    }
+#define BWD2(T, EP_, BITS_)                                                                                          \
+    if (act == kRelu) BWD2_A(T, EP_, kRelu, BITS_) else BWD2_A(T, EP_, kLeaky, BITS_)
+    if (x.sign_bits) {
+        if (E <= 8) BWD2(float, 8, true) else BWD2(float, 16, true)
+    } else if (dtype == DG_DTYPE_BF16) {
+        if (E <= 8) BWD2(bf16_t, 8, false) else BWD2(bf16_t, 16, false)
+    } else {
+        if (E <= 8) BWD2(float, 8, false) else BWD2(float, 16, false)
+    }
+#undef BWD2
+#undef BWD2_A
+#undef BWD2_K
+    if (wg)
+        hipLaunchKernelGGL(embed_finish_kernel, dim3((BwdPart::kTotal + 31) / 32), dim3(1024), 0, stream, part, grid, x.gw1,
+                           static_cast<float*>(nullptr), x.gw2, static_cast<float*>(nullptr), E);
+    return check_launch(who);
+}
+
+}
+
+extern "C" int dg_embed_sym_fwd(const float* a, const float* w1, const float* b1, const float* w2_packed,
+                                const float* b2, void* out, int B, int N, int E, int H, int C, int act, int dtype,
+                                dg_stream_t stream_) {
+    return embed_fwd_impl("dg_embed_sym_fwd", a, w1, b1, w2_packed, b2, out, nullptr, B, N, E, H, C, act, dtype, stream_);
+}
+
+extern "C" int dg_embed_sym_fwd_bits(const float* a, const float* w1, const float* b1, const float* w2_packed,
+                                     const float* b2, void* out, unsigned* sign_bits, int B, int N, int E, int H, int C,
+                                     int act, int dtype, dg_stream_t stream_) {
+    return embed_fwd_impl("dg_embed_sym_fwd_bits", a, w1, b1, w2_packed, b2, out, sign_bits, B, N, E, H, C, act, dtype, stream_);
 }
 
 extern "C" int dg_embed_sym_bwd(const float* a, const float* w1, const float* b1, const float* w2_packed,
@@ -771,46 +939,18 @@
                                 int N, int E, int H, int C, int act, int dtype, dg_stream_t stream_) {
     if (!a || !w1 || !b1 || !w2_packed || !w2_dgrad_packed || !b2 || !g || !dw1 || !db1 || !dw2 || !db2 || !workspace)
         return fail(DG_E_ARG, "dg_embed_sym_bwd: null pointer");
-    if (!dtype_ok(dtype)) return fail(DG_E_ARG, "dg_embed_sym_bwd: unknown dtype %d", dtype);
-    if (B < 1 || !embed_shape_ok(N, E, H, C, act))
-        return fail(DG_E_SHAPE, "dg_embed_sym_bwd: unsupported B=%d N=%d E=%d H=%d C=%d act=%d", B, N, E, H, C, act);
-    if (workspace_bytes < dg_embed_sym_workspace_bytes(B, N))
-        return fail(DG_E_WORKSPACE, "dg_embed_sym_bwd: workspace too small");
-    hipStream_t stream = static_cast<hipStream_t>(stream_);
-    const int tpm = (N * (N + 1) / 2 + kPairs - 1) / kPairs;
-    const int grid = embed_grid(B * tpm, kBwdPerCu);
-    float* part = static_cast<float*>(workspace);
-    constexpr int lds_bytes = (64 * kHid + 64 * kC + 64 * kD1Pitch + 64 * kMaxE + kHid * 16) * 4 + kPairs * 2 * 4;
-    ProfScope prof(DG_K_EMBED_SYM, stream);
-    note_forward(static_cast<int64_t>(B) * N * N);
-#define BWD_D(T, EP_, ACT_, DA_)                                                                                  \
-    {                                                                                                             \
-        DG_OPT_IN_LDS((&embed_sym_bwd_kernel<T, EP_, ACT_, DA_>), lds_bytes);                                      \
-        hipLaunchKernelGGL((embed_sym_bwd_kernel<T, EP_, ACT_, DA_>), dim3(grid), dim3(256), lds_bytes, stream, a, \
-                           w1, b1, w2_packed, w2_dgrad_packed, b2, static_cast<const T*>(g), da, part, B, N, E, tpm); \
-    }
-#define BWD_A(T, EP_, ACT_)                                                                                       \
-    {                                                                                                             \
-        if (da) BWD_D(T, EP_, ACT_, true) else BWD_D(T, EP_, ACT_, false)                                         \
-    }
-#define BWD(T, EP_)                                                                                               \
-    switch (act) {                                                                                                \
-        case kRelu: BWD_A(T, EP_, kRelu) break;                                                                   \
-        case kLeaky: BWD_A(T, EP_, kLeaky) break;                                                                 \
-        case kSigmoid: BWD_A(T, EP_, kSigmoid) break;                                                             \
-        default: BWD_A(T, EP_, kTanh) break;                                                                      \
-    }
-    if (dtype == DG_DTYPE_BF16) {
-        if (E <= 8) BWD(bf16_t, 8) else BWD(bf16_t, 16)
-    } else {
-        if (E <= 8) BWD(float, 8) else BWD(float, 16)
-    }
-#undef BWD_A
-#undef BWD_D
-#undef BWD
-    hipLaunchKernelGGL(embed_finish_kernel, dim3((BwdPart::kTotal + 31) / 32), dim3(1024), 0, stream, part, grid, dw1, db1, dw2,
-                       db2, E);
-    return check_launch("dg_embed_sym_bwd");
+    const dg_embed_bwd_args x{a, w1, b1, w2_packed, w2_dgrad_packed, b2, g, nullptr, da, dw1, db1, dw2, db2,
+                              workspace, workspace_bytes, B, N, E, H, C, act, dtype};
+    return embed_bwd_impl("dg_embed_sym_bwd", x, stream_);
+}
+
+extern "C" int dg_embed_sym_bwd_ex(const dg_embed_bwd_args* x, dg_stream_t stream_) {
+    if (!x) return fail(DG_E_ARG, "dg_embed_sym_bwd_ex: null pointer");
+    const int nw = (x->dw1 != nullptr) + (x->db1 != nullptr) + (x->dw2 != nullptr) + (x->db2 != nullptr);
+    if (!x->a || !x->w1 || !x->b1 || !x->w2_packed || !x->w2_dgrad_packed || !x->b2 || !x->g || (nw == 4 && !x->workspace))
+        return fail(DG_E_ARG, "dg_embed_sym_bwd_ex: null pointer");
+    if (nw != 0 && nw != 4) return fail(DG_E_ARG, "dg_embed_sym_bwd_ex: dw1, db1, dw2, db2 go together");
+    return embed_bwd_impl("dg_embed_sym_bwd_ex", *x, stream_);
 }
 
 extern "C" int dg_embed_sym_bwd2(const float* a, const float* w1, const float* b1, const float* w2_packed,
@@ -819,39 +959,19 @@
                                  int H, int C, int act, int dtype, dg_stream_t stream_) {
     if (!a || !w1 || !b1 || !w2_packed || !w2_dgrad_packed || !b2 || !g || !t || !gg || !gw1 || !gw2 || !workspace)
         return fail(DG_E_ARG, "dg_embed_sym_bwd2: null pointer");
-    if (!dtype_ok(dtype)) return fail(DG_E_ARG, "dg_embed_sym_bwd2: unknown dtype %d", dtype);
-    if (act != kRelu && act != kLeaky)
-        return fail(DG_E_ARG, "dg_embed_sym_bwd2: only piecewise-linear activations (relu, leaky) have this closed form");
-    if (B < 1 || !embed_shape_ok(N, E, H, C, act))
-        return fail(DG_E_SHAPE, "dg_embed_sym_bwd2: unsupported B=%d N=%d E=%d H=%d C=%d act=%d", B, N, E, H, C, act);
-    if (workspace_bytes < dg_embed_sym_workspace_bytes(B, N))
-        return fail(DG_E_WORKSPACE, "dg_embed_sym_bwd2: workspace too small");
-    hipStream_t stream = static_cast<hipStream_t>(stream_);
-    const int tpm = (N * (N + 1) / 2 + kPairs - 1) / kPairs;
-    const int grid = embed_grid(B * tpm, kBwdPerCu);
-    float* part = static_cast<float*>(workspace);
-    constexpr int lds_bytes = (64 * kHid + 64 * kC + 64 * kHid + 2 * 64 * kMaxE + kPairs * kC) * 4 + kPairs * 2 * 4;
-    ProfScope prof(DG_K_EMBED_SYM, stream);
-    note_forward(static_cast<int64_t>(B) * N * N);
-#define BWD2_A(T, EP_, ACT_)                                                                                       \
-    {                                                                                                              \
-        DG_OPT_IN_LDS((&embed_sym_bwd2_kernel<T, EP_, ACT_>), lds_bytes);                                           \
-        hipLaunchKernelGGL((embed_sym_bwd2_kernel<T, EP_, ACT_>), dim3(grid), dim3(256), lds_bytes, stream, a, w1,  \
-                           b1, w2_packed, w2_dgrad_packed, b2, static_cast<const T*>(g), t, static_cast<T*>(gg),   \
-                           part, B, N, E, tpm);                                                                    \
-    }
-#define BWD2(T, EP_)                                                     \
-    if (act == kRelu) BWD2_A(T, EP_, kRelu) else BWD2_A(T, EP_, kLeaky)
-    if (dtype == DG_DTYPE_BF16) {
-        if (E <= 8) BWD2(bf16_t, 8) else BWD2(bf16_t, 16)
-    } else {
-        if (E <= 8) BWD2(float, 8) else BWD2(float, 16)
-    }
-#undef BWD2
-#undef BWD2_A
-    hipLaunchKernelGGL(embed_finish_kernel, dim3((BwdPart::kTotal + 31) / 32), dim3(1024), 0, stream, part, grid, gw1,
-                       static_cast<float*>(nullptr), gw2, static_cast<float*>(nullptr), E);
-    return check_launch("dg_embed_sym_bwd2");
+    const dg_embed_bwd2_args x{a, w1, b1, w2_packed, w2_dgrad_packed, b2, g, t, nullptr, gg, gw1, gw2,
+                               workspace, workspace_bytes, B, N, E, H, C, act, dtype};
+    return embed_bwd2_impl("dg_embed_sym_bwd2", x, stream_);
+}
+
+extern "C" int dg_embed_sym_bwd2_ex(const dg_embed_bwd2_args* x, dg_stream_t stream_) {
+    if (!x) return fail(DG_E_ARG, "dg_embed_sym_bwd2_ex: null pointer");
+    const int nw = (x->gw1 != nullptr) + (x->gw2 != nullptr);
+    if (!x->a || !x->w1 || !x->b1 || !x->w2_packed || !x->w2_dgrad_packed || !x->b2 || !x->g || !x->t || !x->gg ||
+        (nw == 2 && !x->workspace))
+        return fail(DG_E_ARG, "dg_embed_sym_bwd2_ex: null pointer");
+    if (nw == 1) return fail(DG_E_ARG, "dg_embed_sym_bwd2_ex: gw1 and gw2 go together");
+    return embed_bwd2_impl("dg_embed_sym_bwd2_ex", *x, stream_);
 }
 
 extern "C" size_t dg_onehot_embed_workspace_bytes(int E, int C) {
diff --git a/druggen_amd/functional/embed.py b/druggen_amd/functional/embed.py
--- a/druggen_amd/functional/embed.py
+++ b/druggen_amd/functional/embed.py
@@ -1,4 +1,6 @@
 from __future__ import annotations
+
+import ctypes
 
 import torch
 from torch.autograd import Function
@@ -77,6 +79,13 @@
     return _JoinParts.apply(slot, *parts)
 
 
+_PIECEWISE_LINEAR = ("relu", "leaky")
+
+
+def _alloc_sign_bits(words: int, device):
+    return torch.empty(words, dtype=torch.int32, device=device)
+
+
 class _EmbedSym(Function):
     @staticmethod
     def forward(ctx, a, w1, b1, w2, b2, act, out_dtype, slot=None):
@@ -84,42 +93,51 @@
         B, N, _, E = a.shape
         H, C = w1.shape[0], w2.shape[0]
         out = _take_slot(slot, (B, N, N, C), out_dtype, a.device)
-        _lib.launch("dg_embed_sym_fwd", a, _lib.fptr(a), _lib.fptr(_c(w1)), _lib.fptr(_c(b1)),
-                    _lib.fptr(_embed_packed_w2(w2)), _lib.fptr(_c(b2)), _lib.ptr(out), B, N, E, H, C, _ACT_IDS[act],
-                    _lib.dt(out))
-        _account("embed_sym", B * N * N * (4 * E + out.element_size() * C), 2 * B * N * N * (E * H + H * C))
-        ctx.save_for_backward(a, w1, b1, w2, b2)
+        bits = None
+        if (options.embed_sign_bits and act in _PIECEWISE_LINEAR and out_dtype == torch.float32 and B > 0
+                and any(ctx.needs_input_grad[:5])):
+            bits = _alloc_sign_bits(int(_lib.load().dg_embed_sym_sign_words(B, N)), a.device)
+        if bits is None:
+            _lib.launch("dg_embed_sym_fwd", a, _lib.fptr(a), _lib.fptr(_c(w1)), _lib.fptr(_c(b1)),
+                        _lib.fptr(_embed_packed_w2(w2)), _lib.fptr(_c(b2)), _lib.ptr(out), B, N, E, H, C, _ACT_IDS[act],
+                        _lib.dt(out))
+        else:
+            _lib.launch("dg_embed_sym_fwd_bits", a, _lib.fptr(a), _lib.fptr(_c(w1)), _lib.fptr(_c(b1)),
+                        _lib.fptr(_embed_packed_w2(w2)), _lib.fptr(_c(b2)), _lib.ptr(out), bits.data_ptr(), B, N, E, H, C,
+                        _ACT_IDS[act], _lib.dt(out))
+        _account("embed_sym", B * N * N * (4 * E + out.element_size() * C) + (4 * bits.numel() if bits is not None else 0),
+                 2 * B * N * N * (E * H + H * C))
+        ctx.save_for_backward(a, w1, b1, w2, b2, bits)
         ctx.act = act
         ctx.out_dtype = out_dtype
         return out
 
     @staticmethod
     def backward(ctx, g):
-        a, w1, b1, w2, b2 = ctx.saved_tensors
+        a, w1, b1, w2, b2, bits = ctx.saved_tensors
         act = ctx.act
         if torch.is_grad_enabled():
             odt = ctx.out_dtype
             if act in _PIECEWISE_LINEAR:
                 outs = _EmbedSymBwd.apply(a, w1, b1, w2, b2, g, act, odt, ctx.needs_input_grad[0],
-                                          ctx.needs_input_grad[1] and not _inputs_only())
+                                          ctx.needs_input_grad[1] and not _inputs_only(), bits)
                 return tuple(outs) + (None, None, None)
             return _double_backward_fallback(lambda *t: _composite_embed_sym(*t, act).to(odt), (a, w1, b1, w2, b2), g) + (None, None, None)
         return _embed_bwd_launch(a, w1, b1, w2, b2, g, act, ctx.out_dtype, ctx.needs_input_grad[0],
-                                 ctx.needs_input_grad[1] and not _inputs_only()) + (None, None, None)
-
-
-_PIECEWISE_LINEAR = ("relu", "leaky")
-
-
-def _embed_bwd_launch(a, w1, b1, w2, b2, g, act, out_dtype, need_da, need_w):
+                                 ctx.needs_input_grad[1] and not _inputs_only(), bits) + (None, None, None)
+
+
+def _embed_bwd_launch(a, w1, b1, w2, b2, g, act, out_dtype, need_da, need_w, bits=None):
     B, N, _, E = a.shape
     H, C = w1.shape[0], w2.shape[0]
     lib = _lib.load()
+    if not need_da and not need_w:
+        return None, None, None, None, None
     g = _c(g if g.dtype == out_dtype else g.to(out_dtype))
     da = torch.empty_like(a) if need_da else None
-    dw1, db1, dw2, db2 = (torch.empty_like(t) for t in (w1, b1, w2, b2))
     if (out_dtype == torch.bfloat16 and act in _PIECEWISE_LINEAR and E <= 8 and N <= 48
             and options.embed_bf16 == "fast"):
+        dw1, db1, dw2, db2 = (torch.empty_like(t) for t in (w1, b1, w2, b2))
         need = int(lib.dg_embed_sym_bwd_bf16_workspace_bytes(B, N))
         ws = _scratch(a, need, "embed16")
         _lib.launch("dg_embed_sym_bwd_bf16", a, _lib.fptr(a), _lib.fptr(_c(w1)), _lib.fptr(_c(b1)), _lib.fptr(_c(w2)),
@@ -130,53 +148,61 @@
         if not need_w:
             dw1 = db1 = dw2 = db2 = None
         return da, dw1, db1, dw2, db2
-    need = int(lib.dg_embed_sym_workspace_bytes(B, N))
-    ws = _scratch(a, need, "embed")
-    _lib.launch("dg_embed_sym_bwd", a, _lib.fptr(a), _lib.fptr(_c(w1)), _lib.fptr(_c(b1)), _lib.fptr(_embed_packed_w2(w2)),
-                _lib.fptr(_embed_packed_w2(w2, True)), _lib.fptr(_c(b2)), _lib.ptr(g), _lib.ptr(da), _lib.ptr(dw1),
-                _lib.ptr(db1), _lib.ptr(dw2), _lib.ptr(db2), ws.data_ptr(), ws.numel(), B, N, E, H, C, _ACT_IDS[act],
-                _lib.dt(g))
-    _account("embed_sym", B * N * N * (4 * E * (2 if da is not None else 1) + g.element_size() * C),
-             2 * B * N * N * (E * H + H * C) * 3)
-    if not need_w:
-        dw1 = db1 = dw2 = db2 = None
+    dw1, db1, dw2, db2 = (torch.empty_like(t) for t in (w1, b1, w2, b2)) if need_w else (None,) * 4
+    ws = _scratch(a, int(lib.dg_embed_sym_workspace_bytes(B, N)), "embed") if need_w else None
+    if bits is not None and (g.dtype != torch.float32 or act not in _PIECEWISE_LINEAR):
+        bits = None
+    args = _lib.EmbedBwdArgs(_lib.fptr(a), _lib.fptr(_c(w1)), _lib.fptr(_c(b1)), _lib.fptr(_embed_packed_w2(w2)),
+                             _lib.fptr(_embed_packed_w2(w2, True)), _lib.fptr(_c(b2)), _lib.ptr(g),
+                             bits.data_ptr() if bits is not None else None, _lib.ptr(da), _lib.ptr(dw1), _lib.ptr(db1),
+                             _lib.ptr(dw2), _lib.ptr(db2), ws.data_ptr() if need_w else None, ws.numel() if need_w else 0,
+                             B, N, E, H, C, _ACT_IDS[act], _lib.dt(g))
+    _lib.launch("dg_embed_sym_bwd_ex", a, ctypes.byref(args))
+    _account("embed_sym", B * N * N * (4 * E * (2 if da is not None else 1) + g.element_size() * C)
+             + (4 * bits.numel() if bits is not None else 0),
+             2 * B * N * N * (E * H + (0 if bits is not None else H * C) + H * C + (E * H if da is not None else 0)
+                              + (E * H + H * C if need_w else 0)))
     return da, dw1, db1, dw2, db2
 
 
 class _EmbedSymBwd(Function):
 
     @staticmethod
-    def forward(ctx, a, w1, b1, w2, b2, g, act, out_dtype, need_da, need_w):
-        ctx.save_for_backward(a, w1, b1, w2, b2, g)
+    def forward(ctx, a, w1, b1, w2, b2, g, act, out_dtype, need_da, need_w, bits=None):
+        ctx.save_for_backward(a, w1, b1, w2, b2, g, bits)
         ctx.act, ctx.out_dtype = act, out_dtype
         outs = _embed_bwd_launch(a.detach(), w1.detach(), b1.detach(), w2.detach(), b2.detach(), g.detach(), act,
-                                 out_dtype, need_da, need_w)
+                                 out_dtype, need_da, need_w, bits)
         ctx.mark_non_differentiable(*[o for o in outs[1:] if o is not None])
         return outs
 
     @staticmethod
     @torch.autograd.function.once_differentiable
     def backward(ctx, t_da, t_dw1, t_db1, t_dw2, t_db2):
-        a, w1, b1, w2, b2, g = ctx.saved_tensors
+        a, w1, b1, w2, b2, g, bits = ctx.saved_tensors
         if t_da is None:
-            return (None,) * 10
+            return (None,) * 11
         B, N, _, E = a.shape
         H, C = w1.shape[0], w2.shape[0]
         lib = _lib.load()
         g = _c(g if g.dtype == ctx.out_dtype else g.to(ctx.out_dtype))
         t = _c(t_da.float())
         gg = torch.empty_like(g)
-        gw1, gw2 = torch.empty_like(w1), torch.empty_like(w2)
-        need = int(lib.dg_embed_sym_workspace_bytes(B, N))
-        ws = _scratch(a, need, "embed")
-        _lib.launch("dg_embed_sym_bwd2", a, _lib.fptr(_c(a)), _lib.fptr(_c(w1)), _lib.fptr(_c(b1)),
-                    _lib.fptr(_embed_packed_w2(w2)), _lib.fptr(_embed_packed_w2(w2, True)), _lib.fptr(_c(b2)), _lib.ptr(g),
-                    _lib.fptr(t), _lib.ptr(gg), _lib.ptr(gw1), _lib.ptr(gw2), ws.data_ptr(), ws.numel(), B, N, E, H, C,
-                    _ACT_IDS[ctx.act], _lib.dt(g))
-        _account("embed_sym", B * N * N * (8 * E + 2 * g.element_size() * C), 2 * B * N * N * (E * H + H * C) * 4)
-        if _inputs_only() or not ctx.needs_input_grad[1]:
-            gw1 = gw2 = None
-        return None, gw1, None, gw2, None, gg, None, None, None, None
+        need_w = ctx.needs_input_grad[1] and not _inputs_only()
+        gw1, gw2 = (torch.empty_like(w1), torch.empty_like(w2)) if need_w else (None, None)
+        ws = _scratch(a, int(lib.dg_embed_sym_workspace_bytes(B, N)), "embed") if need_w else None
+        if bits is not None and g.dtype != torch.float32:
+            bits = None
+        args = _lib.EmbedBwd2Args(_lib.fptr(_c(a)), _lib.fptr(_c(w1)), _lib.fptr(_c(b1)), _lib.fptr(_embed_packed_w2(w2)),
+                                  _lib.fptr(_embed_packed_w2(w2, True)), _lib.fptr(_c(b2)), _lib.ptr(g), _lib.fptr(t),
+                                  bits.data_ptr() if bits is not None else None, _lib.ptr(gg), _lib.ptr(gw1), _lib.ptr(gw2),
+                                  ws.data_ptr() if need_w else None, ws.numel() if need_w else 0, B, N, E, H, C,
+                                  _ACT_IDS[ctx.act], _lib.dt(g))
+        _lib.launch("dg_embed_sym_bwd2_ex", a, ctypes.byref(args))
+        _account("embed_sym", B * N * N * (8 * E + 2 * g.element_size() * C) + (4 * bits.numel() if bits is not None else 0),
+                 2 * B * N * N * (2 * E * H + H * C + (0 if bits is not None else H * C)
+                                  + (2 * H * C + E * H if need_w else 0)))
+        return None, gw1, None, gw2, None, gg, None, None, None, None, None
 
 
 def embed_sym(a, w1, b1, w2, b2, act: str, out_dtype=torch.float32, slot=None):
diff --git a/druggen_amd/options.py b/druggen_amd/options.py
--- a/druggen_amd/options.py
+++ b/druggen_amd/options.py
@@ -16,6 +16,7 @@
     "ffn_pair": (True, False),
     "penalty_wgrad": ("joined", "engine"),
     "embed_bf16": ("fast", "general"),
+    "embed_sign_bits": (True, False),
 }
 _ENV = {"hidden": "DG_HIDDEN", "ffn_f32": "DG_FFN_F32", "attn_half_f32": "DG_ATTN_HALF_F32",
         "attn_half_f32_bwd": "DG_ATTN_HALF_F32_BWD", "attn_half": "DG_ATTN_HALF", "ffn_bf16": "DG_FFN_BF16",
diff --git a/include/druggen_hip_ext.h b/include/druggen_hip_ext.h
--- /dev/null
+++ b/include/druggen_hip_ext.h
@@ -0,0 +1,36 @@
+#ifndef DRUGGEN_HIP_EXT_H
+#define DRUGGEN_HIP_EXT_H
+
+#include "druggen_hip.h"
+
+#ifdef __cplusplus
+extern "C" {
+#endif
+
+size_t dg_embed_sym_sign_words(int B, int N);
+int dg_embed_sym_fwd_bits(const float* a, const float* w1, const float* b1, const float* w2_packed, const float* b2,
+                          void* out, unsigned* sign_bits, int B, int N, int E, int H, int C, int act, int dtype,
+                          dg_stream_t stream);
+
+typedef struct dg_embed_bwd_args {
+    const float* a; const float* w1; const float* b1; const float* w2_packed; const float* w2_dgrad_packed; const float* b2;
+    const void* g; const unsigned* sign_bits;
+    float* da; float* dw1; float* db1; float* dw2; float* db2;
+    void* workspace; size_t workspace_bytes;
+    int B, N, E, H, C, act, dtype;
+} dg_embed_bwd_args;
+int dg_embed_sym_bwd_ex(const dg_embed_bwd_args* args, dg_stream_t stream);
+
+typedef struct dg_embed_bwd2_args {
+    const float* a; const float* w1; const float* b1; const float* w2_packed; const float* w2_dgrad_packed; const float* b2;
+    const void* g; const float* t; const unsigned* sign_bits;
+    void* gg; float* gw1; float* gw2;
+    void* workspace; size_t workspace_bytes;
+    int B, N, E, H, C, act, dtype;
+} dg_embed_bwd2_args;
+int dg_embed_sym_bwd2_ex(const dg_embed_bwd2_args* args, dg_stream_t stream);
+
+#ifdef __cplusplus
+}
+#endif
+#endif
```

Result: no change. 4934 (median of 6 runs) (+0.4%).
